# ashawkey/nerf2mesh

Hardware: AMD Instinct MI355X
Metric: train_samples_per_sec (higher is better)
Workload: dtype f32 march/composite, f16 autocast encode+MLP (reference -O recipe); 1 GPU; nerf_synthetic/lego stage-0 -O --bound 1 --dt_gamma 0, 800x800 x 100 synthetic views, num_points target 2^18/GPU (adaptive num_rays), occupancy refresh every 16 steps; diffuse_step=1000, refresh_steps_in_window=64, parallelism=single GPU, occupancy_refresh=single GPU, mlp=fused MFMA field kernels, driver=engine.Stage0Engine (fixed launch sequence), pretrain_steps=1000, params=18367240

## Files before the change

### include/n2m_hip.h

```cpp
#ifndef N2M_HIP_H
#define N2M_HIP_H

#include <stdint.h>

#ifdef __cplusplus
extern "C" {
#endif

#define N2M_ABI_VERSION 1

enum { N2M_F32 = 0, N2M_F16 = 1 };

enum {
    N2M_OK = 0,
    N2M_EINVAL = -1,
    N2M_ENULL = -2,
    N2M_EUNSUPPORTED = -3
};

int n2m_abi_version(void);
const char* n2m_last_error(void);


int n2m_near_far_from_aabb(const float* rays_o, const float* rays_d, const float* aabb, uint32_t N,
// ... 368 lines not shown
int n2m_freq_encode_forward(const float* inputs, uint32_t B, uint32_t D, uint32_t deg, uint32_t C,
                            float* outputs, void* stream);
int n2m_freq_encode_backward(const float* grad, const float* outputs, uint32_t B, uint32_t D, uint32_t deg,
                             uint32_t C, float* grad_inputs, void* stream);


int n2m_get_rays(const float* poses, const int64_t* cam, const int64_t* pix, uint32_t N, uint32_t H, uint32_t W,
                 float fx, float fy, float cx, float cy, const float* images, float* rays_o, float* rays_d,
                 float* rgba, void* stream);

int n2m_batch_rays(const float* poses, const float* uniforms, uint32_t V, uint32_t N, uint32_t H, uint32_t W, float fx, float fy, float cx,
                   float cy, const float* images, const float* aabb, float min_near, float* rays_o, float* rays_d, float* rgba,
                   float* nears, float* fars, float* noises, float* bg, int32_t* counter, void* stream);
int n2m_batch_rays_cnf(const float* poses, const float* uniforms, uint32_t V, uint32_t N, uint32_t H, uint32_t W, float fx, float fy, float cx,
                       float cy, const float* images, const float* aabb, float min_near, float* rays_o, float* rays_d, float* rgba,
                       float* nears, float* fars, float* noises, float* bg, int32_t* counter, const float* cam_near_far, void* stream);

int n2m_photo_loss_forward(const float* image, const float* weights_sum, const float* gt_rgba, const float* bg,
                           float bg_scalar, float lambda_rgb, float lambda_mask, uint32_t N, float* partial,
                           uint32_t* ticket, float* loss, void* stream);
int n2m_photo_loss_backward(const float* image, const float* weights_sum, const float* gt_rgba, const float* bg,
                            float bg_scalar, float lambda_rgb, float lambda_mask, uint32_t N,
                            const float* grad_loss, float* d_image, float* d_weights_sum, void* stream);

int n2m_composite_loss_train(const float* sigmas, const float* rgbs, const float* ts, const int32_t* rays, uint32_t M, uint32_t N,
                             float T_thresh, const float* gt_rgba, const float* bg, float bg_scalar, float lambda_rgb, float lambda_mask,
                             const float* grad_loss, float* weights_sum, float* image, float* grad_sigmas, float* grad_rgbs, float* partial,
                             uint32_t* ticket, float* loss, float* loss_sum, void* stream);
int n2m_composite_loss_train_ent(const float* sigmas, const float* rgbs, const float* ts, const int32_t* rays, uint32_t M, uint32_t N,
                                 float T_thresh, const float* gt_rgba, const float* bg, float bg_scalar, float lambda_rgb, float lambda_mask,
                                 const float* grad_loss, float* weights_sum, float* image, float* grad_sigmas, float* grad_rgbs, float* partial,
                                 uint32_t* ticket, float* loss, float* loss_sum, float lambda_entropy, void* stream);
int n2m_composite_loss_train_ex(const float* sigmas, const float* rgbs, const float* ts, const int32_t* rays, uint32_t M, uint32_t N,
                                float T_thresh, const float* gt_rgba, const float* bg, float bg_scalar, float lambda_rgb, float lambda_mask,
                                const float* grad_loss, float* weights_sum, float* image, float* grad_sigmas, float* grad_rgbs, float* partial,
                                uint32_t* ticket, float* loss, float* loss_sum, float lambda_entropy, int alpha_mode, void* stream);

int n2m_composite_live_counts(int32_t* live, uint32_t* block_live);
int n2m_sample_order_live_first(const int32_t* rays, const int32_t* live, const uint32_t* block_live, uint32_t N, uint32_t M,
                                uint32_t* perm, void* stream);
int n2m_grid_backward_sample_order(const uint32_t* perm);

int n2m_grid_backward_merge_levels(uint32_t levels);

#define N2M_ADAM_MAX 16
typedef struct {
    void* param[N2M_ADAM_MAX]; const void* grad[N2M_ADAM_MAX]; void* exp_avg[N2M_ADAM_MAX]; void* exp_avg_sq[N2M_ADAM_MAX];
    void* half_shadow[N2M_ADAM_MAX];
    uint32_t numel[N2M_ADAM_MAX]; float lr[N2M_ADAM_MAX]; int32_t grad_is_half[N2M_ADAM_MAX];
    int32_t shadow_mode[N2M_ADAM_MAX];
    int32_t clear_grad[N2M_ADAM_MAX];
    int32_t slot[N2M_ADAM_MAX];
    uint32_t count;
} N2mAdamDesc;
int n2m_adam_step(const N2mAdamDesc* desc, double beta1, double beta2, float eps, const float* scale,
                  const float* found_inf, const float* bias, void* stream);
#define N2M_EMA_MAX 16
typedef struct {
    void* shadow[N2M_EMA_MAX]; const void* param[N2M_EMA_MAX];
    uint32_t numel[N2M_EMA_MAX];
    uint32_t count;
} N2mEmaDesc;
int n2m_ema_update(const N2mEmaDesc* desc, float one_minus_decay, void* stream);

int n2m_scaler_update(float* scale, float* growth_tracker, float* found_inf, float* step, float* bias, double beta1,
                      double beta2, float growth_factor, float backoff_factor, float growth_interval, void* stream);
int n2m_scaler_update_slots(float* scale, float* growth_tracker, float* found_inf, float* steps, float* bias,
                            uint32_t participants, double beta1, double beta2, float growth_factor, float backoff_factor,
                            float growth_interval, void* stream);

int n2m_scaler_update_slots_loss(float* scale, float* growth_tracker, float* found_inf, float* steps, float* bias,
                                 uint32_t participants, double beta1, double beta2, float growth_factor, float backoff_factor,
                                 float growth_interval, const float* loss_partial, uint32_t n_partial, uint32_t n_rays, float* loss,
                                 float* loss_sum, void* stream);
int n2m_scaler_update_slots_loss2(float* scale, float* growth_tracker, float* found_inf, float* steps, float* bias,
                                  uint32_t participants, double beta1, double beta2, float growth_factor, float backoff_factor,
                                  float growth_interval, const float* loss_partial, uint32_t n_partial, uint32_t n_rays, float* loss,
                                  float* loss_sum, const float* extra_partial, uint32_t n_extra, float extra_scale, void* stream);
int n2m_scaler_update_slots_loss3(float* scale, float* growth_tracker, float* found_inf, float* steps, float* bias,
                                  uint32_t participants, double beta1, double beta2, float growth_factor, float backoff_factor,
                                  float growth_interval, const float* loss_partial, uint32_t n_partial, uint32_t n_rays, float* loss,
                                  float* loss_sum, const float* extra_partial, uint32_t n_extra, float extra_scale,
                                  const float* extra2_partial, uint32_t n_extra2, float extra2_scale, void* stream);

#define N2M_TAIL_TICKET_WORDS (64 * 32)
typedef struct {
    float* growth_tracker; float* steps;
    uint32_t participants; float growth_factor, backoff_factor, growth_interval;
    const float* loss_partial; uint32_t n_partial; uint32_t n_rays; float* loss; float* loss_sum;
    const float* extra_partial; uint32_t n_extra; float extra_scale;
    const float* extra2_partial; uint32_t n_extra2; float extra2_scale;
    uint32_t* ticket;
} N2mScalerTail;
int n2m_adam_step_scaler(const N2mAdamDesc* desc, double beta1, double beta2, float eps, float* scale, float* found_inf, float* bias,
                         const N2mScalerTail* tail, void* stream);

int n2m_sdf_offsets(const float* xyz, uint32_t M, float eps, float bound, float* pts, float* pts01, void* stream);
int n2m_sdf_alpha_forward(const float* sdf, const float* sdf6, const float* dirs, const float* ts, uint32_t M, const float* variance, float eps,
                          float cos_anneal_ratio, float* alpha, float* normal, float* eik_partial, void* stream);
int n2m_sdf_alpha_backward(const float* d_alpha, const float* sdf, const float* sdf6, const float* dirs, const float* ts, uint32_t M,
                           const float* variance, float eps, float cos_anneal_ratio, const float* seed, float eik_coef, float* d_sdf,
                           float* d_sdf6, float* var_partial, float* d_variance, float* found_inf, void* stream);


int n2m_sh_encode_forward(const float* inputs, float* outputs, uint32_t B, uint32_t D, uint32_t degree,
                          float* dy_dx, void* stream);

int n2m_sh_encode_backward(const float* grad, const float* inputs, uint32_t B, uint32_t D, uint32_t degree,
                           const float* dy_dx, float* grad_inputs, void* stream);


enum {
    N2M_K_GRID_FWD = 0, N2M_K_GRID_BWD, N2M_K_GRID_TV, N2M_K_MARCH_COUNT, N2M_K_MARCH_WRITE,
    N2M_K_COMPOSITE_FWD, N2M_K_COMPOSITE_BWD, N2M_K_NEAR_FAR, N2M_K_PACKBITS, N2M_K_MLP_FWD, N2M_K_MLP_BWD,
    N2M_K_RASTER, N2M_K_GRID_FWD_PACKED , N2M_K_ADAM,
    N2M_K_INTERP_FWD, N2M_K_INTERP_BWD, N2M_K_AA_FWD, N2M_K_AA_BWD, N2M_K_RASTER_BWD, N2M_K_COUNT
};
int n2m_prof_enable(int on);
int n2m_prof_reset(void);
int n2m_prof_read(int kernel_id, uint64_t* launches, double* total_ms, double* algo_bytes);
int n2m_prof_seen(int kernel_id, uint64_t* launches_seen);
const char* n2m_prof_name(int kernel_id);

int n2m_stream_copy(const void* src, void* dst, uint64_t bytes, uint32_t workgroups, void* stream);

#ifdef __cplusplus
}
#endif
#endif
```

### include/n2m_mlp.h

```cpp
#ifndef N2M_MLP_H
#define N2M_MLP_H

#include <stdint.h>

#ifdef __cplusplus
extern "C" {
#endif

int n2m_field_forward(const float* xyz, const float* dirs, const float* h1, const void* h2, const float* w_sigma0,
                      const float* w_sigma1, const float* w_color0, const float* w_color1, const float* w_color2,
                      const float* w_spec0, const float* w_spec1, uint32_t M, int shading, int normalize_dirs, float* sigma, float* rgb,
                      float* specular, void* stream);

int n2m_field_backward(const float* xyz, const float* dirs, const float* h1, const void* h2, const float* w_sigma0,
                       const float* w_sigma1, const float* w_color0, const float* w_color1, const float* w_color2,
                       const float* w_spec0, const float* w_spec1, uint32_t M, int shading, int normalize_dirs, const float* d_sigma,
                       const float* d_rgb, const float* d_specular, float* d_h1, void* d_h2, float* d_w_sigma0,
                       float* d_w_sigma1, float* d_w_color0, float* d_w_color1, float* d_w_color2, float* d_w_spec0,
                       float* d_w_spec1, float* found_inf, void* stream);

int n2m_field_forward_train(const float* xyz, const float* dirs, const float* h1, const void* h2, const float* w_sigma0,
                            const float* w_sigma1, const float* w_color0, const float* w_color1, const float* w_color2,
                            const float* w_spec0, const float* w_spec1, uint32_t M, int shading, int normalize_dirs, float* sigma, float* rgb,
                            float* specular, float* spec_sq_partial, void* stream);
int n2m_field_backward_train(const float* xyz, const float* dirs, const float* h1, const void* h2, const float* w_sigma0,
                             const float* w_sigma1, const float* w_color0, const float* w_color1, const float* w_color2,
                             const float* w_spec0, const float* w_spec1, uint32_t M, int shading, int normalize_dirs, const float* d_sigma,
                             const float* d_rgb, const float* d_specular, float* d_h1, void* d_h2, float* d_w_sigma0,
                             float* d_w_sigma1, float* d_w_color0, float* d_w_color1, float* d_w_color2, float* d_w_spec0,
                             float* d_w_spec1, float* found_inf, float spec_reg, const float* seed, void* stream);
uint32_t n2m_field_spec_partials(void);

#ifdef __cplusplus
}
#endif
#endif
```

### nerf2mesh_amd/_lib.py

```python
import ctypes
import os
import threading

_HERE = os.path.dirname(os.path.abspath(__file__))
LIB_PATH = os.environ.get("N2M_HIP_LIB") or os.path.join(_HERE, "lib", "libn2m_hip.so")

_u32, _i32, _f32, _vp, _int, _u64 = ctypes.c_uint32, ctypes.c_int32, ctypes.c_float, ctypes.c_void_p, ctypes.c_int, ctypes.c_uint64

SIGNATURES = {
    "n2m_near_far_from_aabb": [_vp, _vp, _vp, _u32, _f32, _vp, _vp, _vp],
    "n2m_sph_from_ray": [_vp, _vp, _f32, _u32, _vp, _vp],
    "n2m_morton3D": [_vp, _u32, _vp, _vp],
    "n2m_morton3D_invert": [_vp, _u32, _vp, _vp],
    "n2m_packbits": [_vp, _u32, _f32, _vp, _vp],
    "n2m_packbits_dev": [_vp, _u32, _vp, _vp, _vp],
    "n2m_flatten_rays": [_vp, _u32, _u32, _vp, _vp],
    "n2m_march_rays_train": [_vp, _vp, _vp, _f32, _int, _f32, _u32, _u32, _u32, _u32, _vp, _vp, _vp, _vp, _vp, _vp, _vp, _vp, _vp],
    "n2m_march_rays_train_write": [_vp, _vp, _vp, _f32, _int, _f32, _u32, _u32, _u32, _u32, _vp, _vp, _vp, _vp, _vp, _vp, _vp, _u32, _vp],
    "n2m_march_rays_train_fused": [_vp, _vp, _vp, _f32, _int, _f32, _u32, _u32, _u32, _u32, _vp, _vp, _vp, _vp, _vp, _vp, _vp, _vp, _u32, _vp, _u64, _vp],
    "n2m_march_fused_workspace_bytes": [_u32],
    "n2m_march_fallback_count": [_vp],
    "n2m_debug_fill_times": [_int, _vp],
    "n2m_stream_copy": [_vp, _vp, _u64, _u32, _vp],
    "n2m_composite_live_counts": [_vp, _vp],
# ... 33 lines not shown
                                             _vp, _f32, _f32, _f32, _vp, _vp, _f32, _f32, _int, _vp, _u64, _vp],
    "n2m_grid_encode_backward_binned_pair_half": [_vp, _vp, _vp, _vp, _vp, _vp, _u32, _u32, _u32, _f32, _u32, _u32, _int, _u32,
                                                  _vp, _f32, _f32, _f32, _vp, _vp, _f32, _f32, _int, _vp, _u64, _vp, _int],
    "n2m_sdf_fold_plan": [_vp, _u32, _f32, _f32, _u32, _u32, _f32, _u32, _int, _vp, _vp, _vp, _u32, _vp, _u32, _vp],
    "n2m_sdf_fold_gather": [_vp, _u32, _u32, _vp, _vp, _u32, _vp, _u32, _vp, _vp],
    "n2m_grid_encode_backward_binned_lists": [_vp, _vp, _u32, _vp, _vp, _u32, _u32, _u32, _f32, _u32, _u32, _int, _u32, _vp, _int, _vp, _u64, _vp],
    "n2m_grid_encode_backward_binned_pair_fold": [_vp, _vp, _vp, _vp, _vp, _vp, _u32, _u32, _u32, _f32, _u32, _u32, _int, _u32,
                                                  _vp, _f32, _f32, _f32, _vp, _vp, _f32, _f32, _int, _vp, _u64, _vp, _vp, _f32, _f32, _vp],
    "n2m_occupancy_update_partials": [_u32],
    "n2m_occupancy_points": [_vp, _vp, _vp, _f32, _f32, _vp, _u32, _vp],
    "n2m_occupancy_update": [_vp, _vp, _f32, _u32, _f32, _vp, _vp, _vp, _vp, _vp],
    "n2m_grid_pair_fuse_plan": [_u32, _u32, _vp, ctypes.POINTER(ctypes.c_uint32), ctypes.POINTER(ctypes.c_uint32)],
    "n2m_grid_encode_backward_binned_pair_adam": [_vp, _vp, _vp, _vp, _vp, _vp, _u32, _u32, _u32, _f32, _u32, _u32, _int, _u32,
                                                  _vp, _f32, _f32, _f32, _vp, _vp, _f32, _f32, _vp, _u64, _vp, _vp],
    "n2m_adam_fuse_restore": [_vp, _vp, _u32, _vp, _vp],
    "n2m_grid_tv_terms": [_vp, _vp, _vp, _u32, _u32, _f32, _u32, _u32, _int, _u32, _f32, _f32, _f32, _vp, _f32, _f32, _vp, _vp],
    "n2m_grid_encode_backward_binned_pair_tvt": [_vp, _vp, _vp, _vp, _vp, _vp, _u32, _u32, _u32, _f32, _u32, _u32, _int, _u32,
                                                 _vp, _vp, _f32, _f32, _int, _vp, _u64, _vp, _int],
    "n2m_grad_total_variation_binned": [_vp, _vp, _vp, _vp, _f32, _f32, _f32, _vp, _u32, _u32, _u32, _u32, _f32, _u32, _u32, _int, _vp, _u64, _vp],
    "n2m_marching_cubes_workspace_bytes": [_u32, _u32, _u32],
    "n2m_marching_cubes_count": [_vp, _u32, _u32, _u32, ctypes.c_double, _vp, _u64, _vp, _vp],
    "n2m_marching_cubes_emit": [_vp, _u32, _u32, _u32, ctypes.c_double, _vp, _u64, ctypes.c_double, ctypes.c_double, ctypes.c_double, _vp, _int,
                                _u32, _vp, _u32, _vp],
    "n2m_mesh_vertex_flags": [_vp, _u32, _vp, _vp, _vp, _u32, _vp, _vp],
    "n2m_mesh_quadrics": [_vp, _u32, _vp, _vp, _vp, _vp, _vp, ctypes.c_double, _vp, _vp],
    "n2m_mesh_edge_collapse_cost": [_vp, _vp, _vp, _vp, _u32, _vp, _vp, _vp, _vp, _vp, _vp, _int, _vp, _vp, _vp],
    "n2m_mesh_select_collapses": [_vp, _vp, _u32, _vp, _vp, _vp, _u32, _vp, _u64, _vp, _vp, _vp],
    "n2m_mesh_collapse_apply": [_vp, _u32, _vp, _vp, _vp, _vp, _u32, _vp, _u32, _vp, _vp, _vp],
    "n2m_mesh_compact_rows": [_vp, _u32, _u32, _u32, _vp, _vp, _vp, _vp],
    "n2m_mesh_mark_referenced": [_vp, _u32, _u32, _vp, _vp],
    "n2m_mesh_reindex": [_vp, _u32, _vp, _vp],
    "n2m_mesh_subdiv_mark": [_vp, _vp, _u32, _vp, _vp, ctypes.c_double, _u32, _vp, _vp],
    "n2m_mesh_subdiv_midpoints": [_vp, _u32, _vp, _u32, _vp, _vp, _vp],
    "n2m_mesh_subdiv_count": [_vp, _u32, _vp, _vp, _vp],
    "n2m_mesh_subdiv_emit": [_vp, _u32, _vp, _u32, _vp, _vp, _vp, _vp, _vp, _vp, _vp, _vp],
    "n2m_mesh_remesh_split_mark": [_vp, _vp, _u32, _u32, _vp, _vp, ctypes.c_double, _vp, _vp],
    "n2m_mesh_remesh_classify": [_vp, _u32, _vp, _vp, _u32, _vp, _vp, _vp, _vp, _vp, ctypes.c_double, _vp, _vp, _vp],
    "n2m_mesh_remesh_collapse_cost": [_vp, _vp, _vp, _vp, _u32, _vp, _vp, _vp, _vp, _vp, _vp, ctypes.c_double, ctypes.c_double, _vp, _vp, _vp],
    "n2m_mesh_remesh_flip_round": [_vp, _u32, _vp, _vp, _vp, _vp, _u32, _vp, _vp, _vp, _vp, _vp, _vp, _vp, _vp, _vp, _vp, _vp],
    "n2m_mesh_remesh_relax": [_vp, _u32, _vp, _vp, _vp, _vp, _vp, _vp, _vp, _vp, _vp, _vp, _vp],
    "n2m_mesh_remesh_relax_revert": [_vp, _vp, _u32, _vp, _u32, _vp, _vp, _vp, _vp, _vp],
    "n2m_mesh_bvh_morton": [_vp, _vp, _u32] + [ctypes.c_double] * 6 + [_vp, _vp],
    "n2m_mesh_bvh_hierarchy": [_vp, _u32, _vp, _vp, _vp],
    "n2m_mesh_bvh_refit": [_vp, _vp, _vp, _u32, _vp, _vp, _vp, _vp, _vp],
    "n2m_mesh_closest": [_vp, _vp, _vp, _u32, _vp, _vp, _vp, _u32, _int, ctypes.c_double, ctypes.c_double, _vp, _vp, _vp, _vp],
    "n2m_mesh_clean_cell_keys": [_vp, _u32, ctypes.c_double, ctypes.c_double, ctypes.c_double, ctypes.c_double, _i32, _i32, _i32, _vp, _vp],
    "n2m_mesh_clean_merge_round": [_vp, _u32, _vp, _vp, _vp, _i32, _i32, _i32, ctypes.c_double, _vp, _vp, _vp, _vp, _vp],
    "n2m_mesh_clean_repoint": [_vp, _u32, _vp, _vp, _vp],
    "n2m_mesh_clean_dup_null": [_vp, _vp, _u32, _vp, _vp, _vp, _vp],
    "n2m_mesh_clean_components": [_vp, _vp, _u32, _vp, _u32, _vp, _u64, _vp, _vp],
    "n2m_mesh_clean_component_filter": [_u32, _vp, _vp, _u32, _int, ctypes.c_double, _i32, _vp, _vp, _vp],
    "n2m_mesh_clean_nm_edge_init": [_vp, _vp, _u32, _vp, _vp, _vp, _vp, _vp, _vp],
    "n2m_mesh_clean_nm_edge_round": [_u32, _vp, _vp, _vp, _vp, _vp, _vp, _vp, _vp, _vp],
    "n2m_mesh_clean_fan_walk": [_vp, _u32, _u32, _vp, _vp, _vp, _vp, _vp, _vp, _vp, _vp],
    "n2m_mesh_clean_fan_split": [_vp, _u32, _vp, _vp, _vp, _vp, _vp, _u32, _vp],
    "n2m_uv_face_frames": [_vp, _vp, _u32, _vp, _vp, _vp, _vp, _vp, _vp],
    "n2m_uv_edge_faces": [_vp, _u32, _u32, _vp, _vp, _vp],
    "n2m_uv_relax_round": [_u32, _vp, _vp, _vp, _vp, _vp, _vp, _vp, ctypes.c_double, _vp, _vp, _vp, _vp],
    "n2m_uv_charts": [_u32, _vp, _vp, _vp, _vp, _vp, _vp, _vp, _vp, _vp, _vp],
    "n2m_uv_project": [_vp, _vp, _vp, _vp, _u32, _u32, _vp, _vp, _vp],
    "n2m_uv_sum_f64": [_vp, _u32, _vp, _vp],
    "n2m_uv_rects": [_vp, _u32, ctypes.c_double, _i32, _vp, _vp, _vp],
    "n2m_uv_shelf_pack": [_vp, _vp, _u32, _i32, _i32, _vp, _vp, _vp],
    "n2m_uv_write_vt": [_vp, _vp, _vp, _vp, _u32, ctypes.c_double, _i32, _i32, _i32, _vp, _vp],
    "n2m_uv_canvas_evict": [_vp, _vp, _u32, _i32, _i32, _vp, _vp, _vp],
    "n2m_uv_face_metrics": [_vp, _vp, _vp, _u32, _i32, _i32, _vp, _vp, _vp],
    "n2m_texture_pad_nearest": [_vp, _vp, _u32, _u32, _u32, _u32, _vp],
    "n2m_asset_shade": [_vp, _vp, _vp, _vp, _vp, _vp, _vp, _u32, _u32, _u32, _u32, _int, _int, _vp, _vp],
    "n2m_freq_encode_forward": [_vp, _u32, _u32, _u32, _u32, _vp, _vp],
    "n2m_freq_encode_backward": [_vp, _vp, _u32, _u32, _u32, _u32, _vp, _vp],
    "n2m_get_rays": [_vp, _vp, _vp, _u32, _u32, _u32, _f32, _f32, _f32, _f32, _vp, _vp, _vp, _vp, _vp],
    "n2m_batch_rays": [_vp, _vp, _u32, _u32, _u32, _u32, _f32, _f32, _f32, _f32, _vp, _vp, _f32, _vp, _vp, _vp, _vp, _vp, _vp, _vp, _vp, _vp],
    "n2m_batch_rays_cnf": [_vp, _vp, _u32, _u32, _u32, _u32, _f32, _f32, _f32, _f32, _vp, _vp, _f32, _vp, _vp, _vp, _vp, _vp, _vp, _vp, _vp, _vp, _vp],
    "n2m_adam_step": [_vp, ctypes.c_double, ctypes.c_double, _f32, _vp, _vp, _vp, _vp],
    "n2m_adam_step_scaler": [_vp, ctypes.c_double, ctypes.c_double, _f32, _vp, _vp, _vp, _vp, _vp],
    "n2m_ema_update": [_vp, _f32, _vp],
    "n2m_scaler_update": [_vp, _vp, _vp, _vp, _vp, ctypes.c_double, ctypes.c_double, _f32, _f32, _f32, _vp],
    "n2m_scaler_update_slots": [_vp, _vp, _vp, _vp, _vp, _u32, ctypes.c_double, ctypes.c_double, _f32, _f32, _f32, _vp],
    "n2m_scaler_update_slots_loss": [_vp, _vp, _vp, _vp, _vp, _u32, ctypes.c_double, ctypes.c_double, _f32, _f32, _f32, _vp, _u32, _u32, _vp, _vp, _vp],
    "n2m_scaler_update_slots_loss2": [_vp, _vp, _vp, _vp, _vp, _u32, ctypes.c_double, ctypes.c_double, _f32, _f32, _f32, _vp, _u32, _u32, _vp, _vp,
                                      _vp, _u32, _f32, _vp],
    "n2m_scaler_update_slots_loss3": [_vp, _vp, _vp, _vp, _vp, _u32, ctypes.c_double, ctypes.c_double, _f32, _f32, _f32, _vp, _u32, _u32, _vp, _vp,
                                      _vp, _u32, _f32, _vp, _u32, _f32, _vp],
    "n2m_sdf_offsets": [_vp, _u32, _f32, _f32, _vp, _vp, _vp],
    "n2m_sdf_alpha_forward": [_vp, _vp, _vp, _vp, _u32, _vp, _f32, _f32, _vp, _vp, _vp, _vp],
    "n2m_sdf_alpha_backward": [_vp, _vp, _vp, _vp, _vp, _u32, _vp, _f32, _f32, _vp, _f32, _vp, _vp, _vp, _vp, _vp, _vp],
    "n2m_photo_loss_forward": [_vp, _vp, _vp, _vp, _f32, _f32, _f32, _u32, _vp, _vp, _vp, _vp],
    "n2m_photo_loss_backward": [_vp, _vp, _vp, _vp, _f32, _f32, _f32, _u32, _vp, _vp, _vp, _vp],
    "n2m_sh_encode_forward": [_vp, _vp, _u32, _u32, _u32, _vp, _vp],
    "n2m_sh_encode_backward": [_vp, _vp, _u32, _u32, _u32, _vp, _vp, _vp],
    "n2m_field_forward": [_vp] * 11 + [_u32, _int, _int] + [_vp] * 4,
    "n2m_field_backward": [_vp] * 11 + [_u32, _int, _int] + [_vp] * 14,
    "n2m_field_forward_train": [_vp] * 11 + [_u32, _int, _int] + [_vp] * 5,
    "n2m_field_backward_train": [_vp] * 11 + [_u32, _int, _int] + [_vp] * 13 + [_f32, _vp, _vp],
    "n2m_field_spec_partials": [],
    "n2m_rasterize_forward": [_vp, _vp, _u32, _u32, _u32, _u32, _vp, _vp, _vp],
    "n2m_rasterize_backward": [_vp, _vp, _vp, _vp, _u32, _u32, _u32, _u32, _vp, _vp],
    "n2m_interpolate_forward": [_vp, _vp, _vp, _u32, _u32, _u32, _u32, _u32, _vp, _vp],
    "n2m_interpolate_backward": [_vp, _vp, _vp, _vp, _u32, _u32, _u32, _u32, _u32, _vp, _vp, _vp],
    "n2m_interpolate_backward_strided": [_vp, _vp, _vp, _vp, _u32, _u32, _u32, _u32, _u32, _u32, _vp, _vp, _vp],
    "n2m_antialias_build_topology": [_vp, _u32, _vp, _u32, _vp],
    "n2m_antialias_forward": [_vp, _vp, _vp, _vp, _vp, _u32, _u32, _u32, _u32, _u32, _u32, _vp, _vp],
    "n2m_antialias_backward": [_vp, _vp, _vp, _vp, _vp, _u32, _vp, _u32, _u32, _u32, _u32, _u32, _f32, _vp, _vp, _vp],
    "n2m_antialias_backward_seeded": [_vp, _vp, _vp, _vp, _vp, _u32, _vp, _u32, _u32, _u32, _u32, _u32, _f32, _vp, _vp, _vp],
    "n2m_to_clip": [_vp, _vp, _u32, _vp, _vp],
    "n2m_to_clip_backward": [_vp, _vp, _u32, _vp, _vp],
    "n2m_laplacian_forward": [_vp, _vp, _vp, _u32, _vp, _f32, _f32, _f32, _u32, _vp, _vp, _vp, _vp],
    "n2m_laplacian_backward": [_vp, _vp, _vp, _vp, _u32, _vp, _f32, _vp, _f32, _f32, _u32, _vp, _vp, _vp],
    "n2m_laplacian_backward_acc": [_vp, _vp, _vp, _vp, _u32, _vp, _f32, _vp, _f32, _f32, _u32, _vp, _vp, _vp],
    "n2m_gather_rows": [_vp, _vp, _u32, _u32, _vp, _vp],
    "n2m_gather_rows_strided": [_vp, _vp, _u32, _u32, _u32, _vp, _u32, _vp],
    "n2m_scatter_rows_strided": [_vp, _vp, _u32, _u32, _u32, _vp, _u32, _vp],
    "n2m_scatter_rows": [_vp, _vp, _u32, _u32, _vp, _vp],
    "n2m_stage1_head": [_vp, _vp, _vp, _u32, _u32, _u32, _vp, _vp, _f32, _f32, _f32, _vp, _vp, _vp, _vp, _vp, _vp, _vp, _vp, _vp, _vp, _int, _vp, _vp, _vp],
    "n2m_peer_alloc": [ctypes.c_size_t, _int, ctypes.POINTER(_vp)],
    "n2m_peer_free": [_vp],
    "n2m_peer_export": [_vp, _vp],
    "n2m_peer_import": [_vp, ctypes.POINTER(_vp)],
    "n2m_peer_unmap": [_vp],
    "n2m_peer_signal": [_vp, _u32, _vp],
    "n2m_peer_wait": [_vp, _u32, _u32, _u32, _u32, _vp, _vp],
    "n2m_peer_copy": [_vp, _vp, ctypes.c_size_t, _vp],
    "n2m_peer_reduce_slices": [_vp, _vp, _u32, _u32, _vp, _vp, _vp, _vp],
    "n2m_adam_step_peer": [_vp, ctypes.c_double, ctypes.c_double, _f32, _vp, _vp, _vp, _vp, _vp],
    "n2m_grid_backward_peer_route": [_vp],
    "n2m_prof_enable": [_int],
    "n2m_prof_reset": [],
    "n2m_prof_read": [_int, ctypes.POINTER(ctypes.c_uint64), ctypes.POINTER(ctypes.c_double), ctypes.POINTER(ctypes.c_double)],
    "n2m_prof_seen": [_int, ctypes.POINTER(ctypes.c_uint64)],
}

RESTYPES = {"n2m_occupancy_update_partials": _u32, "n2m_grid_binned_workspace_bytes": _u64, "n2m_grid_binned_pair_workspace_bytes": _u64, "n2m_march_fused_workspace_bytes": _u64,
            "n2m_marching_cubes_workspace_bytes": _u64, "n2m_field_spec_partials": _u32}

F32, F16 = 0, 1
ADAM_MAX = 16


class AdamDesc(ctypes.Structure):
    _fields_ = [("param", _vp * ADAM_MAX), ("grad", _vp * ADAM_MAX), ("exp_avg", _vp * ADAM_MAX), ("exp_avg_sq", _vp * ADAM_MAX),
                ("half_shadow", _vp * ADAM_MAX), ("numel", _u32 * ADAM_MAX), ("lr", _f32 * ADAM_MAX), ("grad_is_half", _i32 * ADAM_MAX),
                ("shadow_mode", _i32 * ADAM_MAX), ("clear_grad", _i32 * ADAM_MAX), ("slot", _i32 * ADAM_MAX), ("count", _u32)]


class ScalerTail(ctypes.Structure):
    _fields_ = [("growth_tracker", _vp), ("steps", _vp), ("participants", _u32), ("growth_factor", _f32), ("backoff_factor", _f32),
                ("growth_interval", _f32), ("loss_partial", _vp), ("n_partial", _u32), ("n_rays", _u32), ("loss", _vp), ("loss_sum", _vp),
                ("extra_partial", _vp), ("n_extra", _u32), ("extra_scale", _f32), ("extra2_partial", _vp), ("n_extra2", _u32),
                ("extra2_scale", _f32), ("ticket", _vp)]


EMA_MAX = 16


class EmaDesc(ctypes.Structure):
    _fields_ = [("shadow", _vp * EMA_MAX), ("param", _vp * EMA_MAX), ("numel", _u32 * EMA_MAX), ("count", _u32)]


ASSET_MAX = 8


class AssetTable(ctypes.Structure):
    _fields_ = [("feat0", _vp * ASSET_MAX), ("feat1", _vp * ASSET_MAX), ("Ht", _u32 * ASSET_MAX), ("Wt", _u32 * ASSET_MAX),
                ("face_begin", _u32 * ASSET_MAX), ("count", _u32)]


PEER_MAX = 8


class PeerPtrs(ctypes.Structure):
    _fields_ = [("ptr", _vp * PEER_MAX), ("count", _u32)]


class AdamPeer(ctypes.Structure):
    _fields_ = [("world", _u32), ("slots", (_vp * PEER_MAX) * 16), ("packed_local", _vp), ("packed_remote", _vp * PEER_MAX), ("n_remote", _u32)]


class PeerRoute(ctypes.Structure):
    _fields_ = [("world", _u32), ("split_row", _u32), ("rows_c", _u32), ("rows_f", _u32), ("g1", (_vp * PEER_MAX) * 2), ("g2", (_vp * PEER_MAX) * 2)]


class AdamFuse(ctypes.Structure):
    _fields_ = [("p_in", _vp * 2), ("m_in", _vp * 2), ("v_in", _vp * 2), ("p_out", _vp * 2), ("m_out", _vp * 2), ("v_out", _vp * 2),
                ("packed", _vp), ("first_level", _u32), ("lr", _f32 * 2), ("slot", _i32 * 2), ("beta1", ctypes.c_double),
                ("beta2", ctypes.c_double), ("eps", _f32), ("scale", _vp), ("bias", _vp)]


KERNEL_IDS = {"grid_encode_forward": 0, "grid_encode_backward": 1, "grad_total_variation": 2, "march_rays_train_count": 3,
              "march_rays_train_write": 4, "composite_rays_train_forward": 5, "composite_rays_train_backward": 6,
              "near_far_from_aabb": 7, "packbits": 8, "mlp_forward": 9, "mlp_backward": 10, "rasterize": 11,
              "grid_encode_forward_packed": 12, "adam_step": 13,
              "interpolate_forward": 14, "interpolate_backward": 15, "antialias_forward": 16, "antialias_backward": 17, "rasterize_backward": 18}

_lib = None


def lib():
    global _lib
    if _lib is None:
        import torch
        if not os.path.exists(LIB_PATH):
            raise RuntimeError(
                f"nerf2mesh_amd: {LIB_PATH} is missing -- build it with `python -m nerf2mesh_amd.build` "
                "(hipcc, gfx950). There is no CPU / PyTorch fallback for the hot path.")
        L = ctypes.CDLL(LIB_PATH)
        for name, argtypes in SIGNATURES.items():
            fn = getattr(L, name)
            fn.argtypes = argtypes
            fn.restype = RESTYPES.get(name, ctypes.c_int)
        L.n2m_last_error.restype = ctypes.c_char_p
        L.n2m_prof_name.restype = ctypes.c_char_p
        L.n2m_prof_name.argtypes = [_int]
        L.n2m_abi_version.restype = ctypes.c_int
        if L.n2m_abi_version() != 1:
            raise RuntimeError("nerf2mesh_amd: libn2m_hip.so ABI version mismatch")
        _lib = L
# ... 88 lines not shown
```

### nerf2mesh_amd/backends/__init__.py

```python
import os
import sys


def path():
    return os.path.dirname(os.path.abspath(__file__))


def install(fused_mlp=False):
    if fused_mlp:
        _fuse_on_import()
        track_torch_ema()
    p = path()
    if p not in sys.path:
        sys.path.insert(0, p)
    for name in ("mcubes", "nvdiffrast.torch", "nvdiffrast", "torch_scatter", "_raymarching_mob", "_gridencoder", "_shencoder", "_freqencoder"):
        m = sys.modules.get(name)
        if m is not None and getattr(m, "__n2m_stub__", False):
            del sys.modules[name]
    return p


def fuse_field(cls):
    import torch
    if getattr(cls, "_n2m_fused_field", False):
        return cls
    ref_forward, ref_density = cls.forward, cls.density

    def _prepare(self):
        ok = getattr(self, "_n2m_fuse_ok", None)
        if ok is None:
            try:
                e1, e2 = self.encoder, self.encoder_color
                shapes = [tuple(l.weight.shape) for m in (self.sigma_net, self.color_net, self.specular_net) for l in m.net]
                ok = (not getattr(self.opt, "tcnn", False) and getattr(self, "individual_dim", 0) == 0
                      and all(l.bias is None for m in (self.sigma_net, self.color_net, self.specular_net) for l in m.net)
                      and shapes == [(32, 19), (1, 32), (64, 35), (64, 64), (6, 64), (32, 6), (3, 32)]
                      and e1.embeddings.shape[1] == 1 and e2.embeddings.shape[1] == 2 and e1.num_levels == 16 and e2.num_levels == 16
                      and e1.input_dim == 3 and e2.input_dim == 3)
                if ok:
                    from nerf2mesh_amd.network import NeRFNetwork as _Ours
                    for e in (e1, e2):
                        if not hasattr(e, "host_offsets"):
                            e.host_offsets = [int(v) for v in e.offsets.detach().cpu().tolist()]
                    if not hasattr(type(self), "packed_tables"):
                        type(self).packed_tables = _Ours.packed_tables
                    if not hasattr(type(self), "invalidate_derived_copies"):
                        type(self).invalidate_derived_copies = _Ours.invalidate_derived_copies
                    from nerf2mesh_amd.network import derived_copy_holders
                    derived_copy_holders.add(self)
            except Exception:
                ok = False
            self._n2m_fuse_ok = ok
        return ok

    def forward(self, x, d, c=None, shading="full"):
        if c is None and x.is_cuda and shading in ("full", "diffuse", "specular") and _prepare(self):
            from nerf2mesh_amd.fused import fused_field
            lead = x.shape[:-1]
            sigma, color, specular = fused_field(self, x.reshape(-1, 3), d.reshape(-1, 3), shading)
            return sigma.view(lead), color.view(*lead, 3), (None if specular is None else specular.view(*lead, 3))
        return ref_forward(self, x, d, c, shading)

    def density(self, x):
        if x.is_cuda and not x.requires_grad and _prepare(self):
            from nerf2mesh_amd.fused import fused_density
            return {"sigma": fused_density(self, x.reshape(-1, 3)).view(x.shape[:-1])}
        return ref_density(self, x)

    forward.__doc__ = "nerf2mesh_amd.backends.fuse_field: fused MFMA field when covered, else " + (ref_forward.__qualname__)
    cls.forward, cls.density = forward, density
    cls._n2m_fused_field = True
    cls._n2m_reference_forward, cls._n2m_reference_density = ref_forward, ref_density
    return cls


def track_derived_copies(ema_cls):
    import functools
    if getattr(ema_cls, "_n2m_tracks_derived_copies", False):
        return ema_cls

    def written(ema, parameters):
        if parameters is not None:
            return parameters
        get = getattr(ema, "_get_parameters", None)
        if get is not None:
            return list(get(None))
        for name in ("_params", "params"):
            if isinstance(getattr(ema, name, None), (list, tuple)):
                return list(getattr(ema, name))
        return None

    def wrap(method):
        @functools.wraps(method)
        def wrapped(self, parameters=None):
            if parameters is not None:
                parameters = list(parameters)
            out = method(self, parameters)
            from nerf2mesh_amd.network import derived_copy_holders
            ps = written(self, parameters)
            ids = None if ps is None else {id(p) for p in ps}
            for model in list(derived_copy_holders):
                if ids is None or id(model.encoder.embeddings) in ids or id(model.encoder_color.embeddings) in ids:
                    model.invalidate_derived_copies()
            return out
        return wrapped

    ema_cls.copy_to, ema_cls.restore = wrap(ema_cls.copy_to), wrap(ema_cls.restore)
    ema_cls._n2m_tracks_derived_copies = True
    return ema_cls


def track_torch_ema():
    try:
        import torch_ema
    except ImportError:
        return False
    track_derived_copies(torch_ema.ExponentialMovingAverage)
    return True


def unfuse_field(cls):
    if getattr(cls, "_n2m_fused_field", False):
        cls.forward, cls.density = cls._n2m_reference_forward, cls._n2m_reference_density
        cls._n2m_fused_field = False
    return cls


def _fuse_on_import():
    m = sys.modules.get("nerf.network")
    if m is not None and hasattr(m, "NeRFNetwork"):
        fuse_field(m.NeRFNetwork)
        return
    import importlib.abc
    import importlib.util

    class _Hook(importlib.abc.MetaPathFinder):
        busy = False

        def find_spec(self, name, path_, target=None):
            if name != "nerf.network" or _Hook.busy:
                return None
            _Hook.busy = True
            try:
                spec = importlib.util.find_spec(name)
            finally:
                _Hook.busy = False
            if spec is None or spec.loader is None:
                return None
            loader, exec_module = spec.loader, spec.loader.exec_module

            def patched_exec(module):
                exec_module(module)
                if hasattr(module, "NeRFNetwork"):
                    fuse_field(module.NeRFNetwork)
            try:
                loader.exec_module = patched_exec
            except Exception:
                return None
            return spec

    if not any(type(h).__name__ == "_Hook" for h in sys.meta_path):
        sys.meta_path.insert(0, _Hook())
```

### nerf2mesh_amd/csrc/mlp.hip

```cpp
#include <map>
#include <mutex>

#include "n2m_common.hpp"
#include "../../include/n2m_mlp.h"

namespace {

typedef _Float16 h4 __attribute__((ext_vector_type(4)));
typedef float f16x __attribute__((ext_vector_type(16)));

#define MFMA(a, b, c) __builtin_amdgcn_mfma_f32_32x32x8f16((a), (b), (c), 0, 0, 0)
typedef _Float16 h8 __attribute__((ext_vector_type(8)));
#define MFMA16(a, b, c) __builtin_amdgcn_mfma_f32_32x32x16_f16((a), (b), (c), 0, 0, 0)

constexpr int P_S0 = 28, P_S1 = 36, P_C0 = 44, P_C1 = 68, P_C2 = 68, P_P0 = 12, P_P1 = 36;
constexpr int P_S1T = 12, P_S0T = 36, P_C2T = 12, P_C1T = 68, P_C0T = 68, P_P1T = 12, P_P0T = 36;
constexpr int O_S0 = 0;
constexpr int O_S1 = O_S0 + 32 * P_S0;
constexpr int O_C0 = O_S1 + 32 * P_S1;
constexpr int O_C1 = O_C0 + 64 * P_C0;
constexpr int O_C2 = O_C1 + 64 * P_C1;
constexpr int O_P0 = O_C2 + 32 * P_C2;
constexpr int O_P1 = O_P0 + 32 * P_P0;
constexpr int FWD_HALVES = O_P1 + 32 * P_P1;
constexpr int O_S1T = FWD_HALVES;
constexpr int O_S0T = O_S1T + 32 * P_S1T;
constexpr int O_C2T = O_S0T + 32 * P_S0T;
constexpr int O_C1T = O_C2T + 64 * P_C2T;
constexpr int O_C0T = O_C1T + 64 * P_C1T;
constexpr int O_P1T = O_C0T + 64 * P_C0T;
constexpr int O_P0T = O_P1T + 32 * P_P1T;
constexpr int ALL_W_HALVES = O_P0T + 32 * P_P0T;
constexpr int TILE_PITCH = 68;
constexpr int TILE_HALVES = 32 * TILE_PITCH;
constexpr int BWD_HALVES = ALL_W_HALVES + 4 * 2 * TILE_HALVES;
constexpr int BWD_PC_TILES_HALVES = ALL_W_HALVES + 4 * 4 * TILE_HALVES;
constexpr int BWD_PC_HALVES = BWD_PC_TILES_HALVES > 65536 ? BWD_PC_TILES_HALVES : 65536;

__device__ __forceinline__ int col_color0(int k) { return k < 32 ? 3 + k : (k < 35 ? k - 32 : -1); }
__device__ __forceinline__ int col_sigma0(int k) { return k < 16 ? 3 + k : (k < 19 ? k - 16 : -1); }
__device__ __forceinline__ int col_plain(int k, int in) { return k < in ? k : -1; }

enum Perm { PERM_PLAIN = 0, PERM_COLOR0 = 1, PERM_SIGMA0 = 2 };
__device__ __forceinline__ int col_of(int perm, int k, int in) {
    return perm == PERM_COLOR0 ? col_color0(k) : perm == PERM_SIGMA0 ? col_sigma0(k) : col_plain(k, in);
}

__device__ void stage_w(_Float16* dst, int pitch, const float* __restrict__ W, int out, int in, int m_pad, int k_pad, int perm) {
    for (int idx = threadIdx.x; idx < m_pad * k_pad; idx += blockDim.x) {
        const int m = idx / k_pad, k = idx - m * k_pad;
        const int c = col_of(perm, k, in);
        dst[m * pitch + k] = (_Float16)((m < out && c >= 0) ? W[m * in + c] : 0.0f);
    }
}
__device__ void stage_wt(_Float16* dst, int pitch, const float* __restrict__ W, int out, int in, int m_pad, int k_pad, int perm) {
    for (int idx = threadIdx.x; idx < m_pad * k_pad; idx += blockDim.x) {
        const int m = idx / k_pad, k = idx - m * k_pad;
        const int c = col_of(perm, m, in);
        dst[m * pitch + k] = (_Float16)((k < out && c >= 0) ? W[k * in + c] : 0.0f);
    }
}

struct FieldArgs {
    const float* xyz; const float* dirs; const float* h1; const _Float16* h2;
    const float* w[7];
    uint32_t M; int shading; int normalize_dirs;
    int raw_density;
    float* sigma; float* rgb; float* specular;
    const float* d_sigma; const float* d_rgb; const float* d_specular;
    float* d_h1; _Float16* d_h2; float* dw[7];
    float* found_inf;
    int dbg;
    float* dw_partial;
    float* spec_sq_partial;
    float spec_reg;
    const float* seed;
};
constexpr int kSpecPartials = 512;

template <int PERM>
__device__ __forceinline__ int logical_k(int c) {
    return PERM == PERM_COLOR0 ? (c < 3 ? 32 + c : c - 3) : PERM == PERM_SIGMA0 ? (c < 3 ? 16 + c : c - 3) : c;
}
template <int NT, int OUT, int IN>
struct WRegs { float v[(OUT * IN + NT - 1) / NT]; };
template <int NT, int OUT, int IN>
__device__ __forceinline__ void w_fetch(WRegs<NT, OUT, IN>& r, const float* __restrict__ W) {
#pragma unroll
    for (int i = 0; i < (OUT * IN + NT - 1) / NT; ++i) {
        const int e = (int)threadIdx.x + i * NT;
        r.v[i] = e < OUT * IN ? W[e] : 0.f;
    }
}
template <int NT, int OUT, int IN, int PERM, bool TR>
__device__ __forceinline__ void w_place(const WRegs<NT, OUT, IN>& r, _Float16* fwd, int pitch, _Float16* tr, int pitch_t) {
#pragma unroll
    for (int i = 0; i < (OUT * IN + NT - 1) / NT; ++i) {
        const int e = (int)threadIdx.x + i * NT;
        if (e < OUT * IN) {
            const int m = e / IN, k = logical_k<PERM>(e - m * IN);
            const _Float16 h = (_Float16)r.v[i];
            fwd[m * pitch + k] = h;
            if (TR) tr[k * pitch_t + m] = h;
        }
    }
}
template <int NT, bool TR, bool DO_DENSITY, bool DO_COLOR>
__device__ __forceinline__ void stage_images(_Float16* lds, const FieldArgs& a) {
    WRegs<NT, 32, 19> s0; WRegs<NT, 1, 32> s1; WRegs<NT, 64, 35> c0; WRegs<NT, 64, 64> c1; WRegs<NT, 6, 64> c2; WRegs<NT, 32, 6> p0; WRegs<NT, 3, 32> p1;
    const bool spec = DO_COLOR && a.shading != 0;
    if (DO_DENSITY) { w_fetch(s0, a.w[0]); w_fetch(s1, a.w[1]); }
    if (DO_COLOR) { w_fetch(c0, a.w[2]); w_fetch(c1, a.w[3]); w_fetch(c2, a.w[4]); }
    if (spec) { w_fetch(p0, a.w[5]); w_fetch(p1, a.w[6]); }
    const uint4 z = make_uint4(0u, 0u, 0u, 0u);
    for (int i = threadIdx.x; i < (TR ? ALL_W_HALVES : FWD_HALVES) / 8; i += NT) reinterpret_cast<uint4*>(lds)[i] = z;
    __syncthreads();
    if (DO_DENSITY) {
        w_place<NT, 32, 19, PERM_SIGMA0, TR>(s0, lds + O_S0, P_S0, lds + O_S0T, P_S0T);
        w_place<NT, 1, 32, PERM_PLAIN, TR>(s1, lds + O_S1, P_S1, lds + O_S1T, P_S1T);
    }
    if (DO_COLOR) {
        w_place<NT, 64, 35, PERM_COLOR0, TR>(c0, lds + O_C0, P_C0, lds + O_C0T, P_C0T);
        w_place<NT, 64, 64, PERM_PLAIN, TR>(c1, lds + O_C1, P_C1, lds + O_C1T, P_C1T);
        w_place<NT, 6, 64, PERM_PLAIN, TR>(c2, lds + O_C2, P_C2, lds + O_C2T, P_C2T);
    }
    if (spec) {
        w_place<NT, 32, 6, PERM_PLAIN, TR>(p0, lds + O_P0, P_P0, lds + O_P0T, P_P0T);
        w_place<NT, 3, 32, PERM_PLAIN, TR>(p1, lds + O_P1, P_P1, lds + O_P1T, P_P1T);
    }
    __syncthreads();
}

__device__ __forceinline__ h4 ld_a(const _Float16* W, int pitch, int mb, int kb, int lane) {
    return *reinterpret_cast<const h4*>(W + (32 * mb + (lane & 31)) * pitch + 8 * kb + 4 * (lane >> 5));
}

template <int MB, int KB>
__device__ __forceinline__ void ld_layer(h4 (&w)[MB][KB], const _Float16* W, int pitch, int lane) {
#pragma unroll
    for (int mb = 0; mb < MB; ++mb)
#pragma unroll
        for (int kb = 0; kb < KB; ++kb) w[mb][kb] = ld_a(W, pitch, mb, kb, lane);
}
__device__ __forceinline__ h8 cat8(const h4& lo, const h4& hi) { return __builtin_shufflevector(lo, hi, 0, 1, 2, 3, 4, 5, 6, 7); }
template <int MB, int KB>
__device__ __forceinline__ void mm_layer(f16x (&d)[MB], const h4 (&w)[MB][KB], const h4 (&b)[KB]) {
#pragma unroll
    for (int kb = 0; kb + 1 < KB; kb += 2)
#pragma unroll
        for (int mb = 0; mb < MB; ++mb) d[mb] = MFMA16(cat8(w[mb][kb], w[mb][kb + 1]), cat8(b[kb], b[kb + 1]), d[mb]);
    if (KB & 1) {
#pragma unroll
        for (int mb = 0; mb < MB; ++mb) d[mb] = MFMA(w[mb][KB - 1], b[KB - 1], d[mb]);
    }
}
template <int KB>
__device__ __forceinline__ f16x mm_k(const _Float16* W, int pitch, int mb, const h4 (&b)[KB], f16x acc, int lane) {
#pragma unroll
    for (int kb = 0; kb + 1 < KB; kb += 2)
        acc = MFMA16(cat8(ld_a(W, pitch, mb, kb, lane), ld_a(W, pitch, mb, kb + 1, lane)), cat8(b[kb], b[kb + 1]), acc);
    if (KB & 1) acc = MFMA(ld_a(W, pitch, mb, KB - 1, lane), b[KB - 1], acc);
    return acc;
}

__device__ __forceinline__ h4 zero4() { h4 z = {(_Float16)0, (_Float16)0, (_Float16)0, (_Float16)0}; return z; }
__device__ __forceinline__ f16x zero16() {
    f16x z;
#pragma unroll
    for (int i = 0; i < 16; ++i) z[i] = 0.f;
    return z;
}

typedef _Float16 h2v_t __attribute__((ext_vector_type(2)));
typedef short s2v_t __attribute__((ext_vector_type(2)));
typedef uint32_t u2v_t __attribute__((ext_vector_type(2)));
typedef float f2v_t __attribute__((ext_vector_type(2)));
__device__ __forceinline__ uint32_t cvt_pk(float a, float b) {
    const f2v_t v = {a, b};
    return __builtin_bit_cast(uint32_t, __builtin_convertvector(v, h2v_t));
}
__device__ __forceinline__ uint32_t relu_pk(uint32_t hh) {
    const s2v_t z = {0, 0};
    return __builtin_bit_cast(uint32_t, __builtin_elementwise_max(__builtin_bit_cast(s2v_t, hh), z));
}
__device__ __forceinline__ uint32_t positive_mask(uint32_t relu_out) {
    uint32_t m;
    asm("v_pk_sub_i16 %0, 0, %1\n\tv_pk_ashrrev_i16 %0, 15, %0 op_sel_hi:[0,1]" : "=v"(m) : "v"(relu_out));
    return m;
}
template <int Q>
__device__ __forceinline__ h4 relu_pack(const f16x& d) {
    u2v_t r;
    r.x = relu_pk(cvt_pk(d[4 * Q], d[4 * Q + 1]));
    r.y = relu_pk(cvt_pk(d[4 * Q + 2], d[4 * Q + 3]));
    return __builtin_bit_cast(h4, r);
}
template <int Q>
__device__ __forceinline__ h4 mask_pack(const f16x& d, const h4& fwd) {
    const u2v_t f = __builtin_bit_cast(u2v_t, fwd);
    u2v_t r;
    r.x = cvt_pk(d[4 * Q], d[4 * Q + 1]) & positive_mask(f.x);
    r.y = cvt_pk(d[4 * Q + 2], d[4 * Q + 3]) & positive_mask(f.y);
    return __builtin_bit_cast(h4, r);
}

__device__ __forceinline__ float sigmoid_h(float pre_acc) {
    const float x = (float)(_Float16)pre_acc;
    return (float)(_Float16)(1.0f / (1.0f + expf(-x)));
}


template <typename P>
__device__ __forceinline__ void load_dir(const FieldArgs& a, uint32_t s, P& bp) {
    float d0 = a.dirs[(size_t)s * 3], d1 = a.dirs[(size_t)s * 3 + 1], d2 = a.dirs[(size_t)s * 3 + 2];
    if (a.normalize_dirs) {
// ... 42 lines not shown
    float xyz[3], dir[3], dsig, drgb[3], dspec[3];
};
template <bool DO_DENSITY, bool DO_COLOR, bool BWD>
__device__ __forceinline__ void fetch_tile(const FieldArgs& a, uint32_t tile, int n, int g, RawTile& r) {
    const uint32_t s = tile * 32 + (uint32_t)n;
    const size_t Mz = a.M;
#pragma unroll
    for (int i = 0; i < 8; ++i) { r.h1v[i] = 0.f; r.h2v[i] = 0u; }
#pragma unroll
    for (int i = 0; i < 3; ++i) { r.xyz[i] = 0.f; r.dir[i] = 0.f; r.drgb[i] = 0.f; r.dspec[i] = 0.f; }
    r.dsig = 0.f;
    if (s >= a.M) return;
    if (DO_DENSITY) {
#pragma unroll
        for (int kb = 0; kb < 2; ++kb)
#pragma unroll
            for (int i = 0; i < 4; ++i) r.h1v[4 * kb + i] = a.h1[(size_t)(8 * kb + 4 * g + i) * Mz + s];
    }
    if (DO_COLOR) {
#pragma unroll
        for (int kb = 0; kb < 4; ++kb) {
            r.h2v[2 * kb] = *reinterpret_cast<const uint32_t*>(a.h2 + ((size_t)(4 * kb + 2 * g) * Mz + s) * 2);
            r.h2v[2 * kb + 1] = *reinterpret_cast<const uint32_t*>(a.h2 + ((size_t)(4 * kb + 2 * g + 1) * Mz + s) * 2);
        }
    }
    if (g == 0) {
#pragma unroll
        for (int i = 0; i < 3; ++i) r.xyz[i] = a.xyz[(size_t)s * 3 + i];
        if (DO_COLOR && a.shading != 0) {
#pragma unroll
            for (int i = 0; i < 3; ++i) r.dir[i] = a.dirs[(size_t)s * 3 + i];
        }
        if (BWD) {
            if (DO_DENSITY) r.dsig = a.d_sigma[s];
            if (DO_COLOR) {
#pragma unroll
                for (int i = 0; i < 3; ++i) r.drgb[i] = a.d_rgb[(size_t)s * 3 + i];
                if (a.d_specular && a.shading != 0) {
#pragma unroll
                    for (int i = 0; i < 3; ++i) r.dspec[i] = a.d_specular[(size_t)s * 3 + i];
                }
            }
        }
    }
}
__device__ __forceinline__ void settle_tile(RawTile& r) {
#pragma unroll
    for (int i = 0; i < 8; ++i) { asm volatile("" : "+v"(r.h1v[i])); asm volatile("" : "+v"(r.h2v[i])); }
#pragma unroll
    for (int i = 0; i < 3; ++i) { asm volatile("" : "+v"(r.xyz[i])); asm volatile("" : "+v"(r.dir[i])); asm volatile("" : "+v"(r.drgb[i])); asm volatile("" : "+v"(r.dspec[i])); }
    asm volatile("" : "+v"(r.dsig));
}
__device__ __forceinline__ void density_frags(const RawTile& r, h4 (&b)[3]) {
#pragma unroll
    for (int kb = 0; kb < 2; ++kb)
#pragma unroll
        for (int i = 0; i < 4; ++i) b[kb][i] = (_Float16)r.h1v[4 * kb + i];
    b[2] = zero4();
    b[2][0] = (_Float16)r.xyz[0]; b[2][1] = (_Float16)r.xyz[1]; b[2][2] = (_Float16)r.xyz[2];
}
__device__ __forceinline__ void color_frags(const RawTile& r, h4 (&b)[5]) {
#pragma unroll
    for (int kb = 0; kb < 4; ++kb) {
        const u2v_t v = {r.h2v[2 * kb], r.h2v[2 * kb + 1]};
        b[kb] = __builtin_bit_cast(h4, v);
    }
    b[4] = zero4();
    b[4][0] = (_Float16)r.xyz[0]; b[4][1] = (_Float16)r.xyz[1]; b[4][2] = (_Float16)r.xyz[2];
}
template <typename P>
__device__ __forceinline__ void dir_frag(const FieldArgs& a, const RawTile& r, P& bp) {
    float d0 = r.dir[0], d1 = r.dir[1], d2 = r.dir[2];
    if (a.normalize_dirs) {
        const float nn = sqrtf(fmaxf((d0 * d0 + d1 * d1) + d2 * d2, 1e-20f));
        d0 /= nn; d1 /= nn; d2 /= nn;
    }
    bp[0] = (_Float16)d0; bp[1] = (_Float16)d1; bp[2] = (_Float16)d2;
}

template <bool DO_DENSITY, bool DO_COLOR>
__global__ void __launch_bounds__(256) field_forward_kernel(FieldArgs a) {
    __builtin_amdgcn_s_setprio(3);
    extern __shared__ __attribute__((aligned(16))) _Float16 lds[];
    stage_images<256, false, DO_DENSITY, DO_COLOR>(lds, a);

    const int lane = threadIdx.x & 63, n = lane & 31, g = lane >> 5;
    const uint32_t wave = blockIdx.x * 4 + (threadIdx.x >> 6), n_waves = gridDim.x * 4;
    const uint32_t n_tiles = (a.M + 31) / 32;
    RawTile nxt;
    float spec_sq = 0.f;
    fetch_tile<DO_DENSITY, DO_COLOR, false>(a, wave, n, g, nxt);
    for (uint32_t tile = wave; tile < n_tiles; tile += n_waves) {
        const uint32_t s = tile * 32 + n;
        const bool valid = s < a.M;
        settle_tile(nxt);
        const RawTile cur = nxt;
        fetch_tile<DO_DENSITY, DO_COLOR, false>(a, tile + n_waves, n, g, nxt);
        if (DO_DENSITY) {
            h4 b0[3];
            density_frags(cur, b0);
            f16x d = zero16();
            d = mm_k<3>(lds + O_S0, P_S0, 0, b0, d, lane);
            const h4 b1[4] = {relu_pack<0>(d), relu_pack<1>(d), relu_pack<2>(d), relu_pack<3>(d)};
            f16x o = zero16();
            o = mm_k<4>(lds + O_S1, P_S1, 0, b1, o, lane);
            if (valid && g == 0) a.sigma[s] = a.raw_density ? (float)(_Float16)o[0] : expf((float)(_Float16)o[0]);
        }
        if (DO_COLOR) {
            h4 b0[5];
            color_frags(cur, b0);
            f16x d1[2] = {zero16(), zero16()};
#pragma unroll
            for (int mb = 0; mb < 2; ++mb)
                d1[mb] = mm_k<5>(lds + O_C0, P_C0, mb, b0, d1[mb], lane);
            const h4 b1[8] = {relu_pack<0>(d1[0]), relu_pack<1>(d1[0]), relu_pack<2>(d1[0]), relu_pack<3>(d1[0]),
                              relu_pack<0>(d1[1]), relu_pack<1>(d1[1]), relu_pack<2>(d1[1]), relu_pack<3>(d1[1])};
            f16x d2[2] = {zero16(), zero16()};
#pragma unroll
            for (int mb = 0; mb < 2; ++mb)
                d2[mb] = mm_k<8>(lds + O_C1, P_C1, mb, b1, d2[mb], lane);
            const h4 b2[8] = {relu_pack<0>(d2[0]), relu_pack<1>(d2[0]), relu_pack<2>(d2[0]), relu_pack<3>(d2[0]),
                              relu_pack<0>(d2[1]), relu_pack<1>(d2[1]), relu_pack<2>(d2[1]), relu_pack<3>(d2[1])};
            f16x d3 = zero16();
            d3 = mm_k<8>(lds + O_C2, P_C2, 0, b2, d3, lane);
            const float q0 = sigmoid_h(d3[0]), q1 = sigmoid_h(d3[1]), q2 = sigmoid_h(d3[2]), q3 = sigmoid_h(d3[3]);
            float cr = q0, cg = q1, cb = q2;
            if (a.shading != 0) {
                h4 bp = zero4();
                if (g == 0) {
                    if (valid) dir_frag(a, cur, bp);
                    bp[3] = (_Float16)q3;
                } else { bp[0] = (_Float16)q0; bp[1] = (_Float16)q1; }
                f16x p1 = MFMA(ld_a(lds + O_P0, P_P0, 0, 0, lane), bp, zero16());
                const h4 bq[4] = {relu_pack<0>(p1), relu_pack<1>(p1), relu_pack<2>(p1), relu_pack<3>(p1)};
                f16x p2 = zero16();
                p2 = mm_k<4>(lds + O_P1, P_P1, 0, bq, p2, lane);
                const float s0 = sigmoid_h(p2[0]), s1 = sigmoid_h(p2[1]), s2 = sigmoid_h(p2[2]);
                if (valid && g == 0 && a.specular) {
                    a.specular[(size_t)s * 3] = s0; a.specular[(size_t)s * 3 + 1] = s1; a.specular[(size_t)s * 3 + 2] = s2;
                }
                if (valid && g == 0) spec_sq += (s0 * s0 + s1 * s1) + s2 * s2;
                if (a.shading == 2) { cr = s0; cg = s1; cb = s2; }
                else {
                    cr = fminf(fmaxf((float)(_Float16)(s0 + q0), 0.f), 1.f);
                    cg = fminf(fmaxf((float)(_Float16)(s1 + q1), 0.f), 1.f);
                    cb = fminf(fmaxf((float)(_Float16)(s2 + q2), 0.f), 1.f);
                }
            }
            if (valid && g == 0 && a.rgb) {
                a.rgb[(size_t)s * 3] = cr; a.rgb[(size_t)s * 3 + 1] = cg; a.rgb[(size_t)s * 3 + 2] = cb;
            }
        }
    }
    if (DO_COLOR && a.spec_sq_partial) {
        __shared__ float spec_wave[4];
        const float w = n2m_wave_sum(spec_sq);
        if (lane == 0) spec_wave[threadIdx.x >> 6] = w;
        __syncthreads();
        if (threadIdx.x == 0) a.spec_sq_partial[blockIdx.x] = ((spec_wave[0] + spec_wave[1]) + spec_wave[2]) + spec_wave[3];
        if (blockIdx.x == 0)
            for (int i = (int)gridDim.x + (int)threadIdx.x; i < kSpecPartials; i += 256) a.spec_sq_partial[i] = 0.f;
    }
}

__device__ __forceinline__ void tile_put(_Float16* tile, int kb, const h4& f, int lane) {
    *reinterpret_cast<h4*>(tile + (lane & 31) * TILE_PITCH + 8 * kb + 4 * (lane >> 5)) = f;
}
// ... 279 lines not shown
                if (g == 0) dq3 = (float)(_Float16)dxp[3];
                else { dq0 = (float)(_Float16)dxp[0]; dq1 = (float)(_Float16)dxp[1]; }
            }
            h4 dc = zero4();
            if (g == 0) {
                dc[0] = (_Float16)(dq0 * q0 * (1.f - q0)); dc[1] = (_Float16)(dq1 * q1 * (1.f - q1));
                dc[2] = (_Float16)(dq2 * q2 * (1.f - q2)); dc[3] = (_Float16)(dq3 * q3 * (1.f - q3));
            } else { dc[0] = (_Float16)(dq0 * q0 * (1.f - q0)); dc[1] = (_Float16)(dq1 * q1 * (1.f - q1)); }
            if (!valid) dc = zero4();
            wave_lds_fence();
#pragma unroll
            for (int kb = 0; kb < 8; ++kb) tile_put(tX, kb, b2[kb], lane);
#pragma unroll
            for (int kb = 0; kb < 4; ++kb) tile_put(tY, kb, kb == 0 ? dc : zero4(), lane);
            wave_lds_fence();
            dw_tile<1, 2>(gC2, tY, tX, lane);
            f16x e2[2];
#pragma unroll
            for (int mb = 0; mb < 2; ++mb) e2[mb] = MFMA(ld_a(lds + O_C2T, P_C2T, mb, 0, lane), dc, zero16());
            const h4 dy2[8] = {mask_pack<0>(e2[0], b2[0]), mask_pack<1>(e2[0], b2[1]), mask_pack<2>(e2[0], b2[2]), mask_pack<3>(e2[0], b2[3]),
                               mask_pack<0>(e2[1], b2[4]), mask_pack<1>(e2[1], b2[5]), mask_pack<2>(e2[1], b2[6]), mask_pack<3>(e2[1], b2[7])};
            wave_lds_fence();
#pragma unroll
            for (int kb = 0; kb < 8; ++kb) { tile_put(tX, kb, b1[kb], lane); tile_put(tY, kb, dy2[kb], lane); }
            wave_lds_fence();
            dw_tile<2, 2>(gC1, tY, tX, lane);
            f16x e1[2] = {zero16(), zero16()};
#pragma unroll
            for (int mb = 0; mb < 2; ++mb)
#pragma unroll
                for (int kb = 0; kb < 8; ++kb) e1[mb] = MFMA(ld_a(lds + O_C1T, P_C1T, mb, kb, lane), dy2[kb], e1[mb]);
            const h4 dy1[8] = {mask_pack<0>(e1[0], b1[0]), mask_pack<1>(e1[0], b1[1]), mask_pack<2>(e1[0], b1[2]), mask_pack<3>(e1[0], b1[3]),
                               mask_pack<0>(e1[1], b1[4]), mask_pack<1>(e1[1], b1[5]), mask_pack<2>(e1[1], b1[6]), mask_pack<3>(e1[1], b1[7])};
            wave_lds_fence();
#pragma unroll
            for (int kb = 0; kb < 8; ++kb) { tile_put(tY, kb, dy1[kb], lane); tile_put(tX, kb, kb < 5 ? b0[kb] : zero4(), lane); }
            wave_lds_fence();
            dw_tile<2, 2>(gC0, tY, tX, lane);
            f16x e0 = zero16();
#pragma unroll
            for (int kb = 0; kb < 8; ++kb) e0 = MFMA(ld_a(lds + O_C0T, P_C0T, 0, kb, lane), dy1[kb], e0);
            if (valid) {
                typedef _Float16 h2v __attribute__((ext_vector_type(2)));
#pragma unroll
                for (int r = 0; r < 16; r += 2) {
                    const int row = 8 * (r >> 2) + 4 * g + (r & 3);
                    h2v v;
                    v.x = (_Float16)e0[r]; v.y = (_Float16)e0[r + 1];
                    *reinterpret_cast<h2v*>(a.d_h2 + ((size_t)(row >> 1) * Mz + s) * 2) = v;
                }
            }
        }
    }

    __syncthreads();
    float* stage = reinterpret_cast<float*>(lds);
    auto reduce = [&](auto& acc, int out_pad, int in_pad, float* dW, int out, int in, int k_real, int perm) {
        for (int i = threadIdx.x; i < out_pad * in_pad; i += blockDim.x) stage[i] = 0.f;
        __syncthreads();
        dw_to_lds(stage, in_pad, acc, lane);
        __syncthreads();
        dw_flush(dW, stage, in_pad, out, in, k_real, perm, a.found_inf);
        __syncthreads();
    };
    if (DO_DENSITY) {
        reduce(gS1, 32, 32, a.dw[1], 1, 32, 32, PERM_PLAIN);
        reduce(gS0, 32, 32, a.dw[0], 32, 19, 19, PERM_SIGMA0);
    }
    if (DO_COLOR) {
        reduce(gC2, 32, 64, a.dw[4], 6, 64, 64, PERM_PLAIN);
        reduce(gC1, 64, 64, a.dw[3], 64, 64, 64, PERM_PLAIN);
        reduce(gC0, 64, 64, a.dw[2], 64, 35, 35, PERM_COLOR0);
        if (a.shading != 0) {
            reduce(gP1, 32, 32, a.dw[6], 3, 32, 32, PERM_PLAIN);
            reduce(gP0, 32, 32, a.dw[5], 32, 6, 6, PERM_PLAIN);
        }
    }
}

template <bool DO_DENSITY, bool DO_COLOR>
__global__ void __launch_bounds__(512) __attribute__((amdgpu_waves_per_eu(2, 2))) field_backward_pc_kernel(FieldArgs a) {
    __builtin_amdgcn_s_setprio(3);
    extern __shared__ __attribute__((aligned(16))) _Float16 lds[];
    stage_images<512, true, DO_DENSITY, DO_COLOR>(lds, a);

    const int lane = threadIdx.x & 63, n = lane & 31, g = lane >> 5, wid = threadIdx.x >> 6;
    const int pair = wid & 3;
    const bool producer = wid < 4;
    _Float16* const tbase = lds + ALL_W_HALVES + pair * 4 * TILE_HALVES;
    auto TX = [&](uint32_t st) { return tbase + (st & 1u) * 2 * TILE_HALVES; };
    auto TY = [&](uint32_t st) { return tbase + (st & 1u) * 2 * TILE_HALVES + TILE_HALVES; };
    const uint32_t n_tiles = (a.dbg & 1) ? 0u : (a.M + 31) / 32;
    const size_t Mz = a.M;
    uint32_t st = 0;
    const float spec_k = a.spec_reg != 0.f ? *a.seed * a.spec_reg : 0.f;

    f16x gS0[1][1] = {{zero16()}}, gS1[1][1] = {{zero16()}};
    f16x gC0[2][2], gC1[2][2], gC2[1][2], gP0[1][1] = {{zero16()}}, gP1[1][1] = {{zero16()}};
#pragma unroll
    for (int i = 0; i < 2; ++i)
#pragma unroll
        for (int j = 0; j < 2; ++j) { gC0[i][j] = zero16(); gC1[i][j] = zero16(); gC2[0][j] = zero16(); }

    if (producer) {
    RawTile nxt;
    fetch_tile<DO_DENSITY, DO_COLOR, true>(a, blockIdx.x * 4 + pair, n, g, nxt);
    for (uint32_t base = blockIdx.x * 4; base < n_tiles; base += gridDim.x * 4) {
        const uint32_t tile = base + pair;
        const uint32_t s = tile * 32 + n;
        const bool valid = s < a.M;
        settle_tile(nxt);
        const RawTile cur = nxt;
        fetch_tile<DO_DENSITY, DO_COLOR, true>(a, tile + gridDim.x * 4, n, g, nxt);
        if (DO_DENSITY) {
            h4 b0[3];
            density_frags(cur, b0);
            f16x d = zero16();
            d = mm_k<3>(lds + O_S0, P_S0, 0, b0, d, lane);
            const h4 b1[4] = {relu_pack<0>(d), relu_pack<1>(d), relu_pack<2>(d), relu_pack<3>(d)};
            f16x o = zero16();
            o = mm_k<4>(lds + O_S1, P_S1, 0, b1, o, lane);
            h4 dy1 = zero4();
            if (valid && g == 0) {
                const float pre = (float)(_Float16)o[0];
                dy1[0] = a.raw_density ? (_Float16)cur.dsig : (_Float16)(cur.dsig * expf(fminf(fmaxf(pre, -15.f), 15.f)));
            }
#pragma unroll
            for (int kb = 0; kb < 4; ++kb) { tile_put(TX(st), kb, b1[kb], lane); tile_put(TY(st), kb, kb == 0 ? dy1 : zero4(), lane); }
            __syncthreads(); ++st;
            const f16x dh = MFMA(ld_a(lds + O_S1T, P_S1T, 0, 0, lane), dy1, zero16());
            const h4 dy0[4] = {mask_pack<0>(dh, b1[0]), mask_pack<1>(dh, b1[1]), mask_pack<2>(dh, b1[2]), mask_pack<3>(dh, b1[3])};
#pragma unroll
            for (int kb = 0; kb < 4; ++kb) { tile_put(TY(st), kb, dy0[kb], lane); tile_put(TX(st), kb, kb < 3 ? b0[kb] : zero4(), lane); }
            __syncthreads(); ++st;
            f16x dx = zero16();
            dx = mm_k<4>(lds + O_S0T, P_S0T, 0, dy0, dx, lane);
            if (valid) {
#pragma unroll
                for (int r = 0; r < 8; ++r) {
                    const int row = 8 * (r >> 2) + 4 * g + (r & 3);
                    a.d_h1[(size_t)row * Mz + s] = (float)(_Float16)dx[r];
                }
            }
        }
        if (DO_COLOR) {
            h4 b0[5];
            h4 wC0[2][5], wC1[2][8], wC2[1][8];
            ld_layer(wC0, lds + O_C0, P_C0, lane);
            color_frags(cur, b0);
            ld_layer(wC1, lds + O_C1, P_C1, lane);
            __builtin_amdgcn_sched_barrier(0);
            f16x d1[2] = {zero16(), zero16()};
            mm_layer(d1, wC0, b0);
            ld_layer(wC2, lds + O_C2, P_C2, lane);
            __builtin_amdgcn_sched_barrier(0);
            const h4 b1[8] = {relu_pack<0>(d1[0]), relu_pack<1>(d1[0]), relu_pack<2>(d1[0]), relu_pack<3>(d1[0]),
                              relu_pack<0>(d1[1]), relu_pack<1>(d1[1]), relu_pack<2>(d1[1]), relu_pack<3>(d1[1])};
            f16x d2[2] = {zero16(), zero16()};
            mm_layer(d2, wC1, b1);
            const h4 b2[8] = {relu_pack<0>(d2[0]), relu_pack<1>(d2[0]), relu_pack<2>(d2[0]), relu_pack<3>(d2[0]),
                              relu_pack<0>(d2[1]), relu_pack<1>(d2[1]), relu_pack<2>(d2[1]), relu_pack<3>(d2[1])};
            f16x d3v[1] = {zero16()};
            mm_layer(d3v, wC2, b2);
            const f16x d3 = d3v[0];
            const float q0 = sigmoid_h(d3[0]), q1 = sigmoid_h(d3[1]), q2 = sigmoid_h(d3[2]), q3 = sigmoid_h(d3[3]);

            float gr = 0.f, gg = 0.f, gb = 0.f, es0 = 0.f, es1 = 0.f, es2 = 0.f;
// ... 89 lines not shown
        }
    }
    }
    else
    for (uint32_t base = blockIdx.x * 4; base < n_tiles; base += gridDim.x * 4) {
        if (DO_DENSITY) {
            __syncthreads(); dw_tile<1, 1, true>(gS1, TY(st), TX(st), lane); ++st;
            __syncthreads(); dw_tile<1, 1, true>(gS0, TY(st), TX(st), lane); ++st;
        }
        if (DO_COLOR) {
            if (a.shading != 0) {
                __syncthreads(); dw_tile<1, 1, true>(gP1, TY(st), TX(st), lane); ++st;
                __syncthreads(); dw_tile<1, 1, true>(gP0, TY(st), TX(st), lane); ++st;
            }
            __syncthreads(); dw_tile<1, 2, true>(gC2, TY(st), TX(st), lane); ++st;
            __syncthreads(); dw_tile<2, 2, true>(gC1, TY(st), TX(st), lane); ++st;
            __syncthreads(); dw_tile<2, 2, true>(gC0, TY(st), TX(st), lane); ++st;
        }
    }

    __syncthreads();
    float* stage = reinterpret_cast<float*>(lds);
    float* const part_row = a.dw_partial + (size_t)blockIdx.x * kDwTotal;
    if (a.dbg & 2) return;
    auto put = [&](auto& acc, int base, int out_pad, int in_pad, int total) {
        if (!producer) dw_to_copy(stage + pair * total + base, in_pad, acc, lane);
    };
    auto sum = [&](int base, int total, int in_pad, int mat, int out, int in, int k_real, int perm) {
        dw_store_partial(part_row + kDwOff[mat], stage + base, total, in_pad, out, in, k_real, perm);
    };
    if (DO_COLOR) {
        put(gC1, 0, 64, 64, 8192); put(gC0, 4096, 64, 64, 8192);
        __syncthreads();
        sum(0, 8192, 64, 3, 64, 64, 64, PERM_PLAIN); sum(4096, 8192, 64, 2, 64, 35, 35, PERM_COLOR0);
        __syncthreads();
    }
    constexpr int kSmall = 6144;
    if (DO_COLOR) {
        put(gC2, 0, 32, 64, kSmall);
        if (a.shading != 0) { put(gP1, 4096, 32, 32, kSmall); put(gP0, 5120, 32, 32, kSmall); }
    }
    if (DO_DENSITY) { put(gS1, 2048, 32, 32, kSmall); put(gS0, 3072, 32, 32, kSmall); }
    __syncthreads();
    if (DO_COLOR) {
        sum(0, kSmall, 64, 4, 6, 64, 64, PERM_PLAIN);
        if (a.shading != 0) { sum(4096, kSmall, 32, 6, 3, 32, 32, PERM_PLAIN); sum(5120, kSmall, 32, 5, 32, 6, 6, PERM_PLAIN); }
    }
    if (DO_DENSITY) { sum(2048, kSmall, 32, 1, 1, 32, 32, PERM_PLAIN); sum(3072, kSmall, 32, 0, 32, 19, 19, PERM_SIGMA0); }
}

int check_field(const char* fn, const float* xyz, const float* h1, const float* const* w, bool density, int shading) {
    N2M_REQUIRE(shading >= 0 && shading <= 2, N2M_EINVAL, "%s: shading must be 0 (diffuse), 1 (full) or 2 (specular)", fn);
    N2M_REQUIRE(xyz, N2M_ENULL, "%s: xyz is NULL", fn);
    if (density) N2M_REQUIRE(h1 && w[0] && w[1], N2M_ENULL, "%s: density branch needs h1 and sigma_net weights", fn);
    return 0;
}

float* dw_scratch(hipStream_t s) {
    static std::mutex mu;
    static std::map<std::pair<int, hipStream_t>, float*> bufs;
    std::lock_guard<std::mutex> lk(mu);
    int dev = 0;
    if (hipGetDevice(&dev) != hipSuccess) return nullptr;
    const auto key = std::make_pair(dev, s);
    auto it = bufs.find(key);
    if (it != bufs.end()) return it->second;
    float* p = nullptr;
    if (hipMalloc((void**)&p, (size_t)256 * kDwTotal * sizeof(float)) != hipSuccess) return nullptr;
    bufs[key] = p;
    return p;
}

uint32_t persistent_grid(uint32_t M) {
    const uint32_t tiles = (M + 31) / 32;
    const uint32_t need = (tiles + 3) / 4;
    return need < 256u ? (need ? need : 1u) : 256u;
}

}

static int field_forward_impl(const float* xyz, const float* dirs, const float* h1, const void* h2, const float* w_sigma0,
                                 const float* w_sigma1, const float* w_color0, const float* w_color1, const float* w_color2,
                                 const float* w_spec0, const float* w_spec1, uint32_t M, int shading, int normalize_dirs, float* sigma, float* rgb,
                                 float* specular, float* spec_sq_partial, void* stream) {
    const float* w[7] = {w_sigma0, w_sigma1, w_color0, w_color1, w_color2, w_spec0, w_spec1};
    const bool density = sigma != nullptr;
    if (int rc = check_field("field_forward", xyz, h1, w, density, shading)) return rc;
    const bool color = rgb != nullptr;
    N2M_REQUIRE(density || color, N2M_ENULL, "field_forward: both sigma and rgb are NULL");
    if (color) {
        N2M_REQUIRE(h2 && w[2] && w[3] && w[4], N2M_ENULL, "field_forward: colour branch needs h2 and color_net weights");
        if (shading != 0) N2M_REQUIRE(dirs && w[5] && w[6], N2M_ENULL, "field_forward: shading != 0 needs dirs and specular_net weights");
    }
    if (M == 0) return 0;
    FieldArgs a{};
    a.xyz = xyz; a.dirs = dirs; a.h1 = h1; a.h2 = (const _Float16*)h2; a.normalize_dirs = normalize_dirs & 1; a.raw_density = (normalize_dirs >> 1) & 1;
    for (int i = 0; i < 7; ++i) a.w[i] = w[i];
    a.M = M; a.shading = shading; a.sigma = sigma; a.rgb = rgb; a.specular = specular;
    a.spec_sq_partial = (color && shading != 0) ? spec_sq_partial : nullptr;
    hipStream_t s = (hipStream_t)stream;
    N2M_PROF_K(N2M_K_MLP_FWD, s, (double)M * (12 + 64 + 4 + (color ? 64 + 12 + 12 + 12 : 0)));
    const size_t smem = (size_t)FWD_HALVES * 2;
    if (color && density) N2M_LAUNCH((field_forward_kernel<true, true>), persistent_grid(M) * 2, 256, smem, s, a);
    else if (color) N2M_LAUNCH((field_forward_kernel<false, true>), persistent_grid(M) * 2, 256, smem, s, a);
    else N2M_LAUNCH((field_forward_kernel<true, false>), persistent_grid(M) * 2, 256, smem, s, a);
    N2M_CHECK_LAUNCH();
    return 0;
}

extern "C" int n2m_field_forward(const float* xyz, const float* dirs, const float* h1, const void* h2, const float* w_sigma0,
                                 const float* w_sigma1, const float* w_color0, const float* w_color1, const float* w_color2,
                                 const float* w_spec0, const float* w_spec1, uint32_t M, int shading, int normalize_dirs, float* sigma, float* rgb,
                                 float* specular, void* stream) {
    return field_forward_impl(xyz, dirs, h1, h2, w_sigma0, w_sigma1, w_color0, w_color1, w_color2, w_spec0, w_spec1, M, shading, normalize_dirs,
                              sigma, rgb, specular, nullptr, stream);
}
extern "C" int n2m_field_forward_train(const float* xyz, const float* dirs, const float* h1, const void* h2, const float* w_sigma0,
                                       const float* w_sigma1, const float* w_color0, const float* w_color1, const float* w_color2,
                                       const float* w_spec0, const float* w_spec1, uint32_t M, int shading, int normalize_dirs, float* sigma,
                                       float* rgb, float* specular, float* spec_sq_partial, void* stream) {
    return field_forward_impl(xyz, dirs, h1, h2, w_sigma0, w_sigma1, w_color0, w_color1, w_color2, w_spec0, w_spec1, M, shading, normalize_dirs,
                              sigma, rgb, specular, spec_sq_partial, stream);
}
extern "C" uint32_t n2m_field_spec_partials(void) { return (uint32_t)kSpecPartials; }

static int field_backward_impl(const float* xyz, const float* dirs, const float* h1, const void* h2, const float* w_sigma0,
                                  const float* w_sigma1, const float* w_color0, const float* w_color1, const float* w_color2,
                                  const float* w_spec0, const float* w_spec1, uint32_t M, int shading, int normalize_dirs, const float* d_sigma,
                                  const float* d_rgb, const float* d_specular, float* d_h1, void* d_h2, float* d_w_sigma0,
                                  float* d_w_sigma1, float* d_w_color0, float* d_w_color1, float* d_w_color2, float* d_w_spec0,
                                  float* d_w_spec1, float* found_inf, float spec_reg, const float* seed, void* stream) {
    const float* w[7] = {w_sigma0, w_sigma1, w_color0, w_color1, w_color2, w_spec0, w_spec1};
    float* dw[7] = {d_w_sigma0, d_w_sigma1, d_w_color0, d_w_color1, d_w_color2, d_w_spec0, d_w_spec1};
    const bool density = d_sigma != nullptr;
    if (int rc = check_field("field_backward", xyz, h1, w, density, shading)) return rc;
    if (density) N2M_REQUIRE(d_h1 && dw[0] && dw[1], N2M_ENULL, "field_backward: density gradients are NULL");
    const bool color = d_rgb != nullptr;
    N2M_REQUIRE(density || color, N2M_ENULL, "field_backward: both d_sigma and d_rgb are NULL");
    if (color) {
        N2M_REQUIRE(h2 && d_h2 && w[2] && w[3] && w[4] && dw[2] && dw[3] && dw[4], N2M_ENULL, "field_backward: colour branch tensors are NULL");
        if (shading != 0) N2M_REQUIRE(dirs && w[5] && w[6] && dw[5] && dw[6], N2M_ENULL, "field_backward: specular branch tensors are NULL");
    }
    if (M == 0) return 0;
    static bool attr_set = false;
    if (!attr_set) {
        (void)hipFuncSetAttribute((const void*)field_backward_kernel<true, true>, hipFuncAttributeMaxDynamicSharedMemorySize, BWD_HALVES * 2);
        (void)hipFuncSetAttribute((const void*)field_backward_kernel<true, false>, hipFuncAttributeMaxDynamicSharedMemorySize, BWD_HALVES * 2);
        (void)hipFuncSetAttribute((const void*)field_backward_kernel<false, true>, hipFuncAttributeMaxDynamicSharedMemorySize, BWD_HALVES * 2);
        (void)hipFuncSetAttribute((const void*)field_backward_pc_kernel<true, true>, hipFuncAttributeMaxDynamicSharedMemorySize, BWD_PC_HALVES * 2);
        (void)hipFuncSetAttribute((const void*)field_backward_pc_kernel<true, false>, hipFuncAttributeMaxDynamicSharedMemorySize, BWD_PC_HALVES * 2);
        (void)hipFuncSetAttribute((const void*)field_backward_pc_kernel<false, true>, hipFuncAttributeMaxDynamicSharedMemorySize, BWD_PC_HALVES * 2);
        attr_set = true;
    }
    FieldArgs a{};
    a.xyz = xyz; a.dirs = dirs; a.h1 = h1; a.h2 = (const _Float16*)h2; a.normalize_dirs = normalize_dirs & 1; a.raw_density = (normalize_dirs >> 1) & 1;
    for (int i = 0; i < 7; ++i) { a.w[i] = w[i]; a.dw[i] = dw[i]; }
    a.M = M; a.shading = shading;
    a.spec_reg = (color && shading != 0 && seed) ? spec_reg : 0.f; a.seed = seed;
    a.d_sigma = d_sigma; a.d_rgb = d_rgb; a.d_specular = d_specular; a.d_h1 = d_h1; a.d_h2 = (_Float16*)d_h2; a.found_inf = found_inf;
    static const int dbg = getenv("N2M_FIELD_DEBUG") ? atoi(getenv("N2M_FIELD_DEBUG")) : 0;
    a.dbg = dbg;
    hipStream_t s = (hipStream_t)stream;
    N2M_PROF_K(N2M_K_MLP_BWD, s, (double)M * (12 + 64 + 4 + 64 + (color ? 64 + 12 + 24 + 64 : 0)));
    static const bool single_wave = getenv("N2M_FIELD_BWD_SINGLE") != nullptr;
    if (!single_wave) {
        const size_t smem = (size_t)BWD_PC_HALVES * 2;
        const uint32_t grid = persistent_grid(M);
        float* part = dw_scratch(s);
        N2M_REQUIRE(part != nullptr, (int)hipErrorOutOfMemory, "field_backward: no memory for the weight-gradient scratch");
        a.dw_partial = part;
        if (color && density) N2M_LAUNCH((field_backward_pc_kernel<true, true>), grid, 512, smem, s, a);
        else if (color) N2M_LAUNCH((field_backward_pc_kernel<false, true>), grid, 512, smem, s, a);
        else N2M_LAUNCH((field_backward_pc_kernel<true, false>), grid, 512, smem, s, a);
        N2M_CHECK_LAUNCH();
        DwOut o;
        for (int i = 0; i < 7; ++i) o.dw[i] = dw[i];
        const uint32_t mask = (density ? 0x03u : 0u) | (color ? 0x1Cu : 0u) | (color && shading != 0 ? 0x60u : 0u);
        if (!(dbg & 2)) N2M_LAUNCH(dw_finalize_kernel, (kDwTotal + 63) / 64, 1024, 0, s, part, grid, o, mask, found_inf);
        N2M_CHECK_LAUNCH();
        return 0;
    }
    const size_t smem = (size_t)BWD_HALVES * 2;
    if (color && density) N2M_LAUNCH((field_backward_kernel<true, true>), persistent_grid(M), 256, smem, s, a);
    else if (color) N2M_LAUNCH((field_backward_kernel<false, true>), persistent_grid(M), 256, smem, s, a);
    else N2M_LAUNCH((field_backward_kernel<true, false>), persistent_grid(M), 256, smem, s, a);
    N2M_CHECK_LAUNCH();
    return 0;
}

extern "C" int n2m_field_backward(const float* xyz, const float* dirs, const float* h1, const void* h2, const float* w_sigma0,
                                  const float* w_sigma1, const float* w_color0, const float* w_color1, const float* w_color2,
                                  const float* w_spec0, const float* w_spec1, uint32_t M, int shading, int normalize_dirs, const float* d_sigma,
                                  const float* d_rgb, const float* d_specular, float* d_h1, void* d_h2, float* d_w_sigma0,
                                  float* d_w_sigma1, float* d_w_color0, float* d_w_color1, float* d_w_color2, float* d_w_spec0,
                                  float* d_w_spec1, float* found_inf, void* stream) {
    return field_backward_impl(xyz, dirs, h1, h2, w_sigma0, w_sigma1, w_color0, w_color1, w_color2, w_spec0, w_spec1, M, shading, normalize_dirs,
                               d_sigma, d_rgb, d_specular, d_h1, d_h2, d_w_sigma0, d_w_sigma1, d_w_color0, d_w_color1, d_w_color2, d_w_spec0,
                               d_w_spec1, found_inf, 0.f, nullptr, stream);
}
extern "C" int n2m_field_backward_train(const float* xyz, const float* dirs, const float* h1, const void* h2, const float* w_sigma0,
                                        const float* w_sigma1, const float* w_color0, const float* w_color1, const float* w_color2,
                                        const float* w_spec0, const float* w_spec1, uint32_t M, int shading, int normalize_dirs,
                                        const float* d_sigma, const float* d_rgb, const float* d_specular, float* d_h1, void* d_h2,
                                        float* d_w_sigma0, float* d_w_sigma1, float* d_w_color0, float* d_w_color1, float* d_w_color2,
                                        float* d_w_spec0, float* d_w_spec1, float* found_inf, float spec_reg, const float* seed, void* stream) {
    return field_backward_impl(xyz, dirs, h1, h2, w_sigma0, w_sigma1, w_color0, w_color1, w_color2, w_spec0, w_spec1, M, shading, normalize_dirs,
                               d_sigma, d_rgb, d_specular, d_h1, d_h2, d_w_sigma0, d_w_sigma1, d_w_color0, d_w_color1, d_w_color2, d_w_spec0,
                               d_w_spec1, found_inf, spec_reg, seed, stream);
}
```

### nerf2mesh_amd/csrc/step_helpers.hip

```cpp
#include <string.h>

#include "n2m_common.hpp"
#include "../../include/n2m_peer.h"

namespace {

struct RayTerm {
    float e[3];
    float m;
    float bg[3];
};

__device__ __forceinline__ RayTerm ray_term(const float* __restrict__ image, const float* __restrict__ wsum,
                                            const float* __restrict__ gt, const float* __restrict__ bg, float bg_scalar, uint32_t r) {
    RayTerm t;
    const float4 g = *reinterpret_cast<const float4*>(gt + (size_t)r * 4);
    const float a = g.w, ws = wsum[r];
    const float gc[3] = {g.x, g.y, g.z};
#pragma unroll
    for (int c = 0; c < 3; ++c) {
        t.bg[c] = bg ? bg[(size_t)r * 3 + c] : bg_scalar;
        const float target = gc[c] * a + t.bg[c] * (1.0f - a);
        const float pred = image[(size_t)r * 3 + c] + (1.0f - ws) * t.bg[c];
        t.e[c] = pred - target;
    }
    t.m = ws - a;
    return t;
}

__global__ void __launch_bounds__(256)
photo_loss_forward_kernel(const float* __restrict__ image, const float* __restrict__ wsum, const float* __restrict__ gt,
                          const float* __restrict__ bg, float bg_scalar, float lambda_rgb, float lambda_mask, uint32_t N,
                          float* __restrict__ partial, uint32_t* __restrict__ ticket, float* __restrict__ loss) {
    __shared__ float wave_sum[4];
    __shared__ bool last;
    const uint32_t r = blockIdx.x * 256 + threadIdx.x, lane = threadIdx.x & 63u, wid = threadIdx.x >> 6;
    float l = 0.0f;
    if (r < N) {
        const RayTerm t = ray_term(image, wsum, gt, bg, bg_scalar, r);
        l = lambda_rgb * ((t.e[0] * t.e[0] + t.e[1] * t.e[1] + t.e[2] * t.e[2]) / 3.0f) + lambda_mask * (t.m * t.m);
    }
    l = n2m_wave_sum(l);
    if (lane == 0) wave_sum[wid] = l;
    __syncthreads();
    if (threadIdx.x == 0) {
        partial[blockIdx.x] = (wave_sum[0] + wave_sum[1]) + (wave_sum[2] + wave_sum[3]);
        __threadfence();
        last = atomicAdd(ticket, 1u) == gridDim.x - 1;
    }
    __syncthreads();
    if (last) {
        __threadfence();
        float s = 0.0f;
        for (uint32_t i = threadIdx.x; i < gridDim.x; i += 256) s += __hip_atomic_load(&partial[i], __ATOMIC_RELAXED, __HIP_MEMORY_SCOPE_AGENT);
        s = n2m_wave_sum(s);
        if (lane == 0) wave_sum[wid] = s;
        __syncthreads();
        if (threadIdx.x == 0) {
            *loss = ((wave_sum[0] + wave_sum[1]) + (wave_sum[2] + wave_sum[3])) / (float)N;
            *ticket = 0;
        }
    }
}

__global__ void __launch_bounds__(256)
photo_loss_backward_kernel(const float* __restrict__ image, const float* __restrict__ wsum, const float* __restrict__ gt,
                           const float* __restrict__ bg, float bg_scalar, float lambda_rgb, float lambda_mask, uint32_t N,
                           const float* __restrict__ grad_loss, float* __restrict__ d_image, float* __restrict__ d_wsum) {
    const uint32_t r = blockIdx.x * 256 + threadIdx.x;
    if (r >= N) return;
    const float g = *grad_loss / (float)N;
    const RayTerm t = ray_term(image, wsum, gt, bg, bg_scalar, r);
    float dw = g * lambda_mask * 2.0f * t.m;
#pragma unroll
    for (int c = 0; c < 3; ++c) {
        const float dp = g * lambda_rgb * (2.0f * t.e[c] / 3.0f);
        d_image[(size_t)r * 3 + c] = dp;
        dw -= dp * t.bg[c];
    }
    d_wsum[r] = dw;
}

template <int S>
__global__ void __launch_bounds__(256)
stage1_head_kernel(const float* __restrict__ aa_alpha , const float* __restrict__ aa_rgb ,
// ... 1040 lines not shown
            float acc = 0.0f;
            for (uint32_t i = s; i < n_partial; i += blockDim.x) acc += loss_partial[i];
            acc = n2m_wave_sum(acc);
            if ((s & 63u) == 0u) wave_part[s >> 6] = acc;
        }
        ok = *found_inf == 0.0f;
        __syncthreads();
        if (s == 0) {
            for (uint32_t w = 0; w < (blockDim.x + 63u) / 64u; ++w) {
                if (loss_partial) tot_part += wave_part[w];
                if (extra_partial) tot_extra += wave_extra[w];
                if (extra2_partial) tot_extra2 += wave_extra2[w];
            }
        }
    }
    if (loss_partial && s == 0) {
        float v = tot_part * inv_rays;
        if (extra_partial) v += tot_extra * extra_scale;
        if (extra2_partial) v += tot_extra2 * extra2_scale;
        if (loss) *loss = v;
        if (loss_sum) *loss_sum += v;
    }
    if (s == 0) {
        if (!ok) {
            if (scale) *scale *= backoff_factor;
            if (growth_tracker) *growth_tracker = 0.0f;
        } else if (growth_tracker) {
            const float g = *growth_tracker + 1.0f;
            if (g >= growth_interval) {
                const float ns = *scale * growth_factor;
                if (scale && ns <= 3.0e38f) *scale = ns;
                *growth_tracker = 0.0f;
            } else {
                *growth_tracker = g;
            }
        }
        *found_inf = 0.0f;
    }
    if (s <= N2M_ADAM_MAX) {
        if (ok && (s == 0 || ((participants >> (s - 1u)) & 1u))) steps[s] += 1.0f;
        const double t = (double)steps[s] + 1.0;
        bias[2u * s] = (float)(1.0 - pow(beta1, t));
        bias[2u * s + 1u] = (float)sqrt(1.0 - pow(beta2, t));
    }
}

__global__ void scaler_update_slots_kernel(float* scale, float* growth_tracker, float* found_inf, float* steps ,
                                           float* bias , uint32_t participants, double beta1, double beta2,
                                           float growth_factor, float backoff_factor, float growth_interval,
                                           const float* __restrict__ loss_partial, uint32_t n_partial, float inv_rays,
                                           float* __restrict__ loss, float* __restrict__ loss_sum,
                                           const float* __restrict__ extra_partial, uint32_t n_extra, float extra_scale,
                                           const float* __restrict__ extra2_partial = nullptr, uint32_t n_extra2 = 0, float extra2_scale = 0.0f) {
    __builtin_amdgcn_s_setprio(3);
    scaler_update_slots_body<false>(scale, growth_tracker, found_inf, steps, bias, participants, beta1, beta2, growth_factor, backoff_factor, growth_interval,
                             loss_partial, n_partial, inv_rays, loss, loss_sum, extra_partial, n_extra, extra_scale, extra2_partial, n_extra2, extra2_scale);
}

extern "C" int n2m_scaler_update_slots(float* scale, float* growth_tracker, float* found_inf, float* steps, float* bias,
                                       uint32_t participants, double beta1, double beta2, float growth_factor, float backoff_factor,
                                       float growth_interval, void* stream) {
    N2M_REQUIRE(found_inf != nullptr && steps != nullptr && bias != nullptr, N2M_ENULL, "scaler_update_slots: NULL found_inf / steps / bias");
    scaler_update_slots_kernel<<<1, 64, 0, (hipStream_t)stream>>>(scale, growth_tracker, found_inf, steps, bias, participants, beta1, beta2,
                                                                  growth_factor, backoff_factor, growth_interval, nullptr, 0u, 0.0f, nullptr, nullptr, nullptr, 0u, 0.0f);
    N2M_CHECK_LAUNCH();
    return 0;
}

extern "C" int n2m_scaler_update_slots_loss3(float* scale, float* growth_tracker, float* found_inf, float* steps, float* bias,
                                            uint32_t participants, double beta1, double beta2, float growth_factor, float backoff_factor,
                                            float growth_interval, const float* loss_partial, uint32_t n_partial, uint32_t n_rays, float* loss,
                                            float* loss_sum, const float* extra_partial, uint32_t n_extra, float extra_scale, const float* extra2_partial,
                                             uint32_t n_extra2, float extra2_scale, void* stream) {
    N2M_REQUIRE(found_inf != nullptr && steps != nullptr && bias != nullptr, N2M_ENULL, "scaler_update_slots: NULL found_inf / steps / bias");
    N2M_REQUIRE(loss_partial != nullptr && n_rays > 0, N2M_EINVAL, "scaler_update_slots_loss: needs the loss partials and the ray count");
    scaler_update_slots_kernel<<<1, 256, 0, (hipStream_t)stream>>>(scale, growth_tracker, found_inf, steps, bias, participants, beta1, beta2,
                                                                  growth_factor, backoff_factor, growth_interval, loss_partial, n_partial,
                                                                  1.0f / (float)n_rays, loss, loss_sum, extra_partial, extra_partial ? n_extra : 0u, extra_scale,
                                                                  extra2_partial, extra2_partial ? n_extra2 : 0u, extra2_scale);
    N2M_CHECK_LAUNCH();
    return 0;
}

extern "C" int n2m_scaler_update_slots_loss2(float* scale, float* growth_tracker, float* found_inf, float* steps, float* bias,
                                             uint32_t participants, double beta1, double beta2, float growth_factor, float backoff_factor,
                                             float growth_interval, const float* loss_partial, uint32_t n_partial, uint32_t n_rays, float* loss,
                                             float* loss_sum, const float* extra_partial, uint32_t n_extra, float extra_scale, void* stream) {
    return n2m_scaler_update_slots_loss3(scale, growth_tracker, found_inf, steps, bias, participants, beta1, beta2, growth_factor, backoff_factor,
                                         growth_interval, loss_partial, n_partial, n_rays, loss, loss_sum, extra_partial, n_extra, extra_scale,
                                         nullptr, 0u, 0.0f, stream);
}

extern "C" int n2m_scaler_update_slots_loss(float* scale, float* growth_tracker, float* found_inf, float* steps, float* bias,
                                            uint32_t participants, double beta1, double beta2, float growth_factor, float backoff_factor,
                                            float growth_interval, const float* loss_partial, uint32_t n_partial, uint32_t n_rays, float* loss,
                                            float* loss_sum, void* stream) {
    return n2m_scaler_update_slots_loss2(scale, growth_tracker, found_inf, steps, bias, participants, beta1, beta2, growth_factor, backoff_factor,
                                         growth_interval, loss_partial, n_partial, n_rays, loss, loss_sum, nullptr, 0u, 0.0f, stream);
}

extern "C" int n2m_scaler_update(float* scale, float* growth_tracker, float* found_inf, float* step, float* bias, double beta1,
                                 double beta2, float growth_factor, float backoff_factor, float growth_interval, void* stream) {
    N2M_REQUIRE(found_inf != nullptr, N2M_ENULL, "scaler_update: found_inf is NULL");
    scaler_update_kernel<<<1, 1, 0, (hipStream_t)stream>>>(scale, growth_tracker, found_inf, step, bias, beta1, beta2, growth_factor,
                                                           backoff_factor, growth_interval);
    N2M_CHECK_LAUNCH();
    return 0;
}

struct EmaTensors {
    uint64_t shadow[N2M_EMA_MAX], param[N2M_EMA_MAX];
    uint32_t n[N2M_EMA_MAX], first_block[N2M_EMA_MAX + 1];
    uint32_t count;
};

__global__ void __launch_bounds__(256) ema_update_kernel(EmaTensors t, float one_minus_decay) {
    uint32_t k = 0;
    while (k + 1 < t.count && blockIdx.x >= t.first_block[k + 1]) ++k;
    const uint32_t i0 = ((blockIdx.x - t.first_block[k]) * 256u + threadIdx.x) * 4u;
    const uint32_t n = t.n[k];
    if (i0 >= n) return;
    float* __restrict__ S = reinterpret_cast<float*>(t.shadow[k]);
    const float* __restrict__ P = reinterpret_cast<const float*>(t.param[k]);
    typedef float f4v __attribute__((ext_vector_type(4)));
    if (i0 + 4u <= n && (((t.shadow[k] | t.param[k]) & 15u) == 0)) {
        f4v s = __builtin_nontemporal_load(reinterpret_cast<const f4v*>(S + i0));
        const f4v p = __builtin_nontemporal_load(reinterpret_cast<const f4v*>(P + i0));
        s.x = s.x - (s.x - p.x) * one_minus_decay; s.y = s.y - (s.y - p.y) * one_minus_decay;
        s.z = s.z - (s.z - p.z) * one_minus_decay; s.w = s.w - (s.w - p.w) * one_minus_decay;
        __builtin_nontemporal_store(s, reinterpret_cast<f4v*>(S + i0));
    } else {
        for (uint32_t e = 0; e < 4u && i0 + e < n; ++e) S[i0 + e] = S[i0 + e] - (S[i0 + e] - P[i0 + e]) * one_minus_decay;
    }
}

extern "C" int n2m_ema_update(const N2mEmaDesc* d, float one_minus_decay, void* stream) {
    N2M_REQUIRE(d != nullptr, N2M_ENULL, "ema_update: NULL descriptor");
    N2M_REQUIRE(d->count >= 1 && d->count <= N2M_EMA_MAX, N2M_EINVAL, "ema_update: 1..%d tensors per call (got %u)", N2M_EMA_MAX, d->count);
    N2M_REQUIRE(one_minus_decay >= 0.0f && one_minus_decay <= 1.0f, N2M_EINVAL, "ema_update: 1 - decay = %g outside [0, 1]", (double)one_minus_decay);
    EmaTensors t;
    t.count = d->count;
    uint32_t blocks = 0;
    for (uint32_t k = 0; k < d->count; ++k) {
        N2M_REQUIRE(d->shadow[k] && d->param[k], N2M_ENULL, "ema_update: NULL tensor %u", k);
        N2M_REQUIRE((((uintptr_t)d->shadow[k] | (uintptr_t)d->param[k]) & 3u) == 0, N2M_EINVAL, "ema_update: tensor %u is not 4-byte aligned", k);
        N2M_REQUIRE(d->shadow[k] != d->param[k], N2M_EINVAL, "ema_update: tensor %u: shadow and parameter are the same memory", k);
        t.shadow[k] = (uint64_t)(uintptr_t)d->shadow[k];
        t.param[k] = (uint64_t)(uintptr_t)d->param[k];
        t.n[k] = d->numel[k];
        t.first_block[k] = blocks;
        blocks += (d->numel[k] + 1023u) / 1024u;
    }
    t.first_block[d->count] = blocks;
    if (blocks == 0) return 0;
    ema_update_kernel<<<blocks, 256, 0, (hipStream_t)stream>>>(t, one_minus_decay);
    N2M_CHECK_LAUNCH();
    return 0;
}
```

### nerf2mesh_amd/engine.py

```python
import ctypes
import os
import time

import numpy as np
import torch

from . import _lib as L
from . import raymarching, synthetic
from .fused import SHADING, _affine
from .gridencoder import _host_offsets, same_geometry
from .optim import FusedAdamAMP

_p = L.ptr


def _shard_refresh_default():
    from .parallel import shard_refresh_default
    return shard_refresh_default()


def lr_lambda(it, iters):
    return 0.01 + 0.99 * (it / 500) if it <= 500 else 0.1 ** ((it - 500) / (iters - 500))


# ... 18 lines not shown
        self.one_pass = False
        self.host_count = torch.empty(1, dtype=torch.int32, pin_memory=True)
        self.count_ready = torch.cuda.Event()
        self.written = torch.cuda.Event()
        self.spec = False
        self.index = 0
        self.M = None
        self.loss = torch.empty(1, dtype=torch.float32, device=dev)
        self.samples = None
        self.cap_m = 0
        self.N = 0
        self.args = None
        self.refreshed = False


class Stage0Engine:
    def __init__(self, model, opt, poses, device, rank=0, world_size=1, seed=0, ema_decay=0.95):
        self.model, self.opt, self.device = model.to(device), opt, torch.device(device)
        dev = self.device
        assert dev.type == "cuda", "the step executor drives HIP kernels: no CPU path"
        if bool(opt.sdf) and world_size > 1:
            raise ValueError("Stage0Engine runs the SDF recipe on one rank; use trainer.Stage0Trainer for multi-rank SDF training")
        if not self.supported(model, opt):
            raise ValueError("Stage0Engine covers the fused recipes (fused_mlp, fp16, no individual codes, power-of-two "
                             "bound, shared encoder geometry); use trainer.Stage0Trainer for other configurations")
        L.lib()
        self.poses = poses.to(dev).float().contiguous()
        self.rank, self.world = rank, world_size
        self.global_step = 0
        self.num_rays = opt.num_rays
        self.gen = torch.Generator(device=dev)
        self.gen.manual_seed(seed + rank)
        self.optimizer = FusedAdamAMP(model.get_params(opt.lr), eps=1e-15, amp=True)
        self.ema = None
        self.epoch_len = max(1, int(poses.shape[0]))
        if ema_decay is not None:
            from .ema import ExponentialMovingAverage
            self.ema = ExponentialMovingAverage(model.parameters(), decay=ema_decay)
        self.images = None
        self.scene = getattr(opt, "scene", "lego")
        self.boxes = synthetic.boxes(dev, self.scene)
        self.cam_near_far = synthetic.cam_near_far(self.poses, self.scene) if getattr(opt, "enable_cam_near_far", False) else None
        self.samples_seen = self.rays_seen = 0
        self.last_num_points = 0
        self._loss_pending, self._loss_sum = [], torch.zeros(1, device=dev)
        self.sync = None
        if world_size > 1:
            from .parallel import GradSync
            self.sync = GradSync(model, world_size)
            self.model.refresh_shard = (rank, world_size) if _shard_refresh_default() else None
        self.side = L.side_stream(dev, slot=2)
        self.tv_stream = L.side_stream(dev, slot=3, priority=int(os.environ.get("N2M_TV_PRIO", "0")))
        self.tv_split = os.environ.get("N2M_TV_SPLIT", "0") == "1"
        self.tv_at = int(os.environ.get("N2M_TV_AT", "0"))
        self.split_backward = True
        self.overlap = True
        self.single_pass = os.environ.get("N2M_MARCH_PASSES", "1") != "2"
        self.marker_at = int(os.environ.get("N2M_MARKER_AT", "0"))
        self.tv_corners = (os.environ.get("N2M_TV_CORNERS", "0") == "1" and world_size == 1 and not opt.sdf and opt.lambda_tv > 0
                           and not self.tv_split)
        self.tv_fwd = (os.environ.get("N2M_TV_FWD", "1") != "0" and world_size == 1 and not opt.sdf and opt.lambda_tv > 0
                       and not self.tv_split and not self.tv_corners)
        self.adam_tail = os.environ.get("N2M_ADAM_TAIL", "0") == "1" and world_size == 1
        self._tail_ticket = torch.zeros(64 * 32, dtype=torch.int32, device=dev)
        self._mid_events = None
        self.live_first = os.environ.get("N2M_LIVE_FIRST", "0") not in ("0", "")
        self._identity_order = os.environ.get("N2M_LIVE_FIRST", "0") == "2"
        self.lookup_overlap = os.environ.get("N2M_LOOKUP_OVERLAP", "0") == "1" and world_size == 1 and not opt.sdf
        self._fine_ready = None
        if self.lookup_overlap:
            self.s_lookup = L.side_stream(dev, slot=4)
        if os.environ.get("N2M_FILL_DBG"):
            L.call("n2m_debug_fill_times", int(os.environ["N2M_FILL_DBG"]), None)

        e1, e2 = model.encoder, model.encoder_color
        self.rows = e1.embeddings.shape[0]
        self.Lv = e1.num_levels
        self.S = float(np.log2(e1.per_level_scale))
        self.H0 = int(e1.base_resolution)
        self.ho = _host_offsets(e1)
        self.aff = _affine(float(model.bound))
        self.mlp_params = [p for m in (model.sigma_net, model.color_net, model.specular_net) for p in m.parameters()]
        assert len(self.mlp_params) == 7
        self.g1 = torch.empty(self.rows, 1, dtype=torch.float32, device=dev)
        self.g2 = torch.empty(self.rows, 2, dtype=torch.float16, device=dev)
        self.dw = torch.zeros(sum(p.numel() for p in self.mlp_params), dtype=torch.float32, device=dev)
        self.dw_views, o = [], 0
        for p in self.mlp_params:
            self.dw_views.append(self.dw[o:o + p.numel()])
            o += p.numel()
        self._desc = {}
        self._bufs = [None, None, None]
        self._marker = None
        self._last = None
        self._queue = []
        self._prepared = 0
        self.depth = 2
        self._cur = 0

        self._work_cap = (0, 0)
        self._n_spec = int(L.lib().n2m_field_spec_partials())
        self._ticket = torch.zeros(1, dtype=torch.int32, device=dev)
        self._seed = None
        self._aabb = None
        self.shard = False
        if world_size > 1:
            import torch.distributed as dist
            W, split = world_size, int(self.ho[8]) if self.Lv == 16 else 0
            fine = self.rows - split
            peer_mode = os.environ.get("N2M_PEER_STORE", "0") == "1" and not opt.sdf
            cs = split // W
            self._uneven = False
            padded = peer_chunk_rows(split, W, int(os.environ.get("N2M_PEER_PAD_ROWS", "0"))) if peer_mode else None
            if padded is not None:
                cs, even_ok = padded, True
                self._uneven = cs * W != split
            else:
                even_ok = split % W == 0
            ok = self.Lv == 16 and even_ok and fine % W == 0 and os.environ.get("N2M_SHARD_ADAM", "1") != "0"
            if ok:
                self.shard = True
                self._split, self._Cs, self._Fs = split, cs, fine // W
                f32 = lambda *sh: torch.empty(*sh, dtype=torch.float32, device=dev)
                f16 = lambda *sh: torch.empty(*sh, dtype=torch.float16, device=dev)
                self.g1s = {"c": f32(self._Cs, 1), "f": f32(self._Fs, 1)}
                self.g2s = {"c": f16(self._Cs, 2), "f": f16(self._Fs, 2)}
                self._inplace_gather = dist.get_backend() == "nccl"
                self.chunked_gather = os.environ.get("N2M_CHUNKED_GATHER", "1") != "0"
        self._bwd_cfg = (2 if self.shard else 1, float(world_size))
        self.peer = None
        if self.shard and os.environ.get("N2M_PEER_STORE", "0") == "1":
            if opt.sdf:
                raise ValueError("N2M_PEER_STORE covers the NeRF recipes (the SDF head's folded backward is not routed)")
            from .parallel import PeerExchange
            self.peer = PeerExchange(rank, world_size, self.rows, self._split, self._Cs, self._Fs, dev, small_n=self.dw.numel() + 1)
            self._peer_small = torch.empty(self.dw.numel() + 1, dtype=torch.float32, device=dev)
            pk = model.packed_tables()
            self.peer.packed.copy_(pk)
            model._packed = self.peer.packed
            model._packed_buffer = self.peer.packed
            self._peer_route = self.peer.route()
            self._peer_fused = (os.environ.get("N2M_PEER_FUSED", "1") != "0" and self._Cs % 4 == 0 and self._Fs % 4 == 0 and self._split % 2 == 0)
            self._adam_peer = None
        if self.shard:
            self.optimizer.shard_sync = lambda: self.sync_parameters(moments=True)
        self.sdf_fold = os.environ.get("N2M_SDF_FOLD", "1") != "0"
        self.sdf_tv_all = os.environ.get("N2M_SDF_TV_ALL", "1") != "0"
        self.fuse_adam = None
        if world_size == 1 and not opt.sdf and self.Lv == 16 and os.environ.get("N2M_FUSE_ADAM", "0") == "1":
            fl, fr = ctypes.c_uint32(0), ctypes.c_uint32(0)
            self._fuse_cap = 1 << 19
            L.call("n2m_grid_pair_fuse_plan", self._fuse_cap, self.Lv, self.ho.ctypes.data, ctypes.byref(fl), ctypes.byref(fr))
            if fl.value < self.Lv:
                self.fuse_adam = {"first_level": int(fl.value), "first_row": int(fr.value), "alt": None, "desc": {}}
                self._bwd_cfg = (2, 1.0)

    @staticmethod
    def supported(model, opt):
        e1, e2 = model.encoder, model.encoder_color
        sdf = bool(opt.sdf)
        return (bool(getattr(opt, "fused_mlp", False)) and bool(opt.fp16) and getattr(opt, "ind_dim", 0) == 0
                and _affine(float(model.bound)) is not None and same_geometry(e1, e2) and e1.embeddings.shape[1] == 1
                and e2.embeddings.shape[1] == 2 and (sdf or not getattr(opt, "progressive_level", False))
                and opt.patch_size == 1 and (sdf or model.max_level >= e1.num_levels) and not (sdf and opt.lambda_entropy > 0))

    @property
# ... 301 lines not shown
                desc.param[k], desc.grad[k] = p.data_ptr() + off, g.data_ptr()
                desc.exp_avg[k], desc.exp_avg_sq[k] = st["exp_avg"].data_ptr() + off, st["exp_avg_sq"].data_ptr() + off
                desc.half_shadow[k], desc.shadow_mode[k] = pk.data_ptr() + row0 * 8, mode
                desc.numel[k], desc.grad_is_half[k], desc.clear_grad[k] = n * C, is_half, 0
                desc.slot[k] = o._slot[p]
                participants |= 1 << (o._slot[p] - 1)
                groups.append(group_of[p])
                k += 1
        live = set(self.mlp_params[:5]) | (set(self.mlp_params[5:]) if full else set())
        views = dict(zip(self.mlp_params, self.dw_views))
        for p in params:
            if p not in live:
                continue
            st = o.state[p]
            desc.param[k], desc.grad[k] = p.data_ptr(), views[p].data_ptr()
            desc.exp_avg[k], desc.exp_avg_sq[k] = st["exp_avg"].data_ptr(), st["exp_avg_sq"].data_ptr()
            desc.half_shadow[k], desc.shadow_mode[k] = None, 0
            desc.numel[k], desc.grad_is_half[k], desc.clear_grad[k] = p.numel(), 0, 1
            desc.slot[k] = o._slot[p]
            participants |= 1 << (o._slot[p] - 1)
            groups.append(group_of[p])
            k += 1
        desc.count = k
        d = self._desc[key] = (desc, participants, groups)
        return d

    def _gather_packed(self):
        import torch.distributed as dist
        flat = self._packed.view(-1)
        self._gathers = {}
        for h in ("c", "f"):
            row0, n = self._shard_ranges()[h]
            lo = 0 if h == "c" else self._split
            out = flat[lo * 2:(lo + self.world * n) * 2]
            mine = flat[row0 * 2:(row0 + n) * 2]
            self._gathers[h] = dist.all_gather_into_tensor(out, mine if self._inplace_gather else mine.clone(), async_op=True)
        if not self.chunked_gather:
            self._wait_gather()

    def _wait_gather(self, which=("c", "f")):
        g = getattr(self, "_gathers", None)
        if not g:
            return
        for h in which:
            w = g.pop(h, None)
            if w is not None:
                w.wait()

    @torch.no_grad()
    def sync_parameters(self, density_only=False, moments=False):
        if not self.shard:
            return
        self._wait_gather()
        if self.peer is not None:
            self.peer.check()
        done = getattr(self, "_synced", (-1, False, False))
        level = (not density_only, moments)
        if done[0] == self.global_step and (done[1] or density_only) and (done[2] or not moments):
            return
        self._synced = (self.global_step, level[0] or (done[0] == self.global_step and done[1]), level[1] or (done[0] == self.global_step and done[2]))
        import torch.distributed as dist
        e1p, e2p = self.model.encoder.embeddings, self.model.encoder_color.embeddings
        tables = [(e1p.data, 1)] if density_only else [(e1p.data, 1), (e2p.data, 2)]
        if moments:
            for p, C in ((e1p, 1), (e2p, 2)):
                st = self.optimizer.state[p]
                tables += [(st["exp_avg"], C), (st["exp_avg_sq"], C)]
        for t, C in tables:
            flat = t.view(-1)
            for h, (row0, n) in self._shard_ranges().items():
                lo = 0 if h == "c" else self._split
                if h == "c" and getattr(self, "_uneven", False):
                    for r in range(self.world):
                        r0, rn = self._shard_ranges_of(r)["c"]
                        if rn > 0:
                            dist.broadcast(flat[r0 * C:(r0 + rn) * C], src=r)
                    continue
                dist.all_gather_into_tensor(flat[lo * C:(lo + self.world * n) * C], flat[row0 * C:(row0 + n) * C].clone())

    def _optimizer_step(self, full, lr_factor, loss_out=None, fused=None):
        o = self.optimizer
        self._wait_gather()
        desc, participants, groups = self._adam_desc(full, dense_only=fused is not None)
        for k, gi in enumerate(groups):
            desc.lr[k] = float(o.param_groups[gi]["initial_lr"]) * lr_factor
        b1, b2 = o.param_groups[0]["betas"]
        s = L.stream()
        peer_fused = self.peer is not None and self._peer_fused
        scaler_done = False
        if self.lookup_overlap and fused is None and not self.shard and self.Lv == 16:
            d_f, d_c = self._adam_desc_halves(full, lr_factor)
            for d in (d_f, d_c):
                L.call("n2m_adam_step", ctypes.addressof(d), float(b1), float(b2), float(o.param_groups[0]["eps"]), _p(o.scale), _p(o.found_inf),
                       _p(o.bias), s)
                if d is d_f:
                    self._fine_ready = torch.cuda.Event()
                    self._fine_ready.record()
        elif peer_fused:
            if self._adam_peer is None:
                self._adam_peer = self.peer.adam_peer([("s1", "c"), ("s2", "c"), ("s1", "f"), ("s2", "f")] + [None] * (desc.count - 4))
            L.call("n2m_adam_step_peer", ctypes.addressof(desc), float(b1), float(b2), float(o.param_groups[0]["eps"]), _p(o.scale), _p(o.found_inf),
                   _p(o.bias), ctypes.addressof(self._adam_peer), s)
        elif (self.adam_tail and loss_out is not None and fused is None and self.peer is None and not self.shard):
            gf, bf, gi = o.growth
            n_rays, buf, extra = loss_out[:3]
            extra2 = loss_out[3] if len(loss_out) > 3 else None
            ex_buf, ex_scale = extra if extra is not None else (None, 0.0)
            e2_buf, e2_n, e2_scale = extra2 if extra2 is not None else (None, 0, 0.0)
            tail = L.ScalerTail(_p(o.growth_tracker), _p(o.steps), participants, gf, bf, gi, _p(self._w["partial"]), (n_rays + 15) // 16, n_rays,
                                _p(buf), _p(self._loss_sum), _p(ex_buf), self._n_spec, float(ex_scale), _p(e2_buf), int(e2_n), float(e2_scale),
                                _p(self._tail_ticket))
            L.call("n2m_adam_step_scaler", ctypes.addressof(desc), float(b1), float(b2), float(o.param_groups[0]["eps"]), _p(o.scale), _p(o.found_inf),
                   _p(o.bias), ctypes.addressof(tail), s)
            scaler_done = True
        else:
            L.call("n2m_adam_step", ctypes.addressof(desc), float(b1), float(b2), float(o.param_groups[0]["eps"]), _p(o.scale), _p(o.found_inf),
                   _p(o.bias), s)
        self.model.encoder_color._half_version = -1
        if fused is not None:
            L.call("n2m_adam_fuse_restore", ctypes.addressof(fused), self.ho.ctypes.data, self.Lv, _p(o.found_inf), s)
            self._fuse_swap()
        if self.peer is not None:
            for h, (row0, n) in self._shard_ranges().items():
                if peer_fused:
                    self.peer.signal_rows(h)
                else:
                    self.peer.push_rows(h, row0, n)
            self._gathers = self.peer.rows_tokens()
            if not self.chunked_gather:
                self._wait_gather()
        elif self.shard:
            self._gather_packed()
        gf, bf, gi = o.growth
        if scaler_done:
            pass
        elif loss_out is None:
            L.call("n2m_scaler_update_slots", _p(o.scale), _p(o.growth_tracker), _p(o.found_inf), _p(o.steps), _p(o.bias), participants,
                   float(b1), float(b2), gf, bf, gi, s)
        else:
            n_rays, buf, extra = loss_out[:3]
            extra2 = loss_out[3] if len(loss_out) > 3 else None
            ex_buf, ex_scale = extra if extra is not None else (None, 0.0)
            e2_buf, e2_n, e2_scale = extra2 if extra2 is not None else (None, 0, 0.0)
            L.call("n2m_scaler_update_slots_loss3", _p(o.scale), _p(o.growth_tracker), _p(o.found_inf), _p(o.steps), _p(o.bias), participants,
                   float(b1), float(b2), gf, bf, gi, _p(self._w["partial"]), (n_rays + 15) // 16, n_rays, _p(buf), _p(self._loss_sum),
                   _p(ex_buf), self._n_spec, float(ex_scale), _p(e2_buf), int(e2_n), float(e2_scale), s)
        nxt = lr_lambda(self.global_step, self.opt.iters)
        for group in o.param_groups:
            group["lr"] = float(group["initial_lr"]) * nxt

    @torch.no_grad()
    def train_step(self):
        opt, model, dev = self.opt, self.model, self.device
        if not model.training:
            model.train()
        for g in self.optimizer.param_groups:
            g.setdefault("initial_lr", g["lr"])
        if not self._queue:
            self._fill_pipeline()
        b = self._queue.pop(0)
        self.global_step += 1
        assert b.index == self.global_step
        N = b.N
        random_bg = b.bg is not None
        bg = b.bg
        shading = SHADING["diffuse" if (self.global_step < opt.diffuse_step or opt.diffuse_only) else "full"]
        M = self._finish(b)
        self.last_num_points = M
        self.samples_seen += M
        self.rays_seen += N

        if opt.sdf:
            opt.cos_anneal_ratio = min(1, self.global_step / (0.5 * opt.iters))
            opt.normal_anneal_epsilon = 1e-1 * (1 - min(0.999, self.global_step / (0.5 * opt.iters)))
            if opt.progressive_level:
                model.max_level = 4 + int(12 * min(1, self.global_step / (0.5 * opt.iters)))
        w = self._work(max(M, 1), N)
        s = L.stream()
        c = b.cap_m
        xyzs = dirs = ts = None
        if M > 0:
            xyzs, dirs, ts = b.samples[:3 * c], b.samples[3 * c:6 * c], b.samples[6 * c:]
        o = self.optimizer
        pk = model.packed_tables()
        if self.lookup_overlap and getattr(self, "_packed", None) is not None and pk.data_ptr() != self._packed.data_ptr():
            self._fine_ready = None
        sw = self.mlp_params
        e1 = model.encoder
        seed = o.scale if self.world == 1 else o.scale / self.world
        if opt.sdf:
            return self._step_sdf(b, M, N, w, xyzs, dirs, ts, shading, seed, pk)
        fwd_terms = False
        if M > 0:
            fwd = (_p(xyzs), _p(pk), _p(e1.offsets), _p(w["h1"]), _p(w["h2"]), M, self.Lv, self.Lv, self.S, self.H0, e1.gridtype_id,
                   int(bool(e1.align_corners)), e1.interp_id, float(self.aff[0]), float(self.aff[1]))
            if self.shard and getattr(self, "_gathers", None) and self.Lv == 16:
                self._wait_gather(("c",))
                L.call("n2m_grid_encode_forward_packed_levels", *fwd, 0, 8, s)
                self._wait_gather(("f",))
                L.call("n2m_grid_encode_forward_packed_levels", *fwd, 8, 8, s)
            elif self.lookup_overlap and self._fine_ready is not None and self.Lv == 16:
                self.s_lookup.wait_event(self._fine_ready)
                with torch.cuda.stream(self.s_lookup):
                    L.call("n2m_grid_encode_forward_packed_levels", *fwd, 8, 8, L.stream())
                    done = torch.cuda.Event()
                    done.record()
                L.call("n2m_grid_encode_forward_packed_levels", *fwd, 0, 8, s)
                torch.cuda.current_stream(dev).wait_event(done)
            elif self.tv_corners and self.Lv == 16 and self.fuse_adam is None:
                L.call("n2m_grid_encode_forward_packed_tv", *fwd, _p(w["tv4"]), s)
                self._corners_of = (self.global_step, M)
            elif self.tv_fwd and self.Lv == 16 and self.fuse_adam is None:
                L.call("n2m_grid_encode_forward_packed_tvterms", *fwd, float(opt.lambda_tv), float(opt.lambda_tv * (10 if opt.bound > 1 else 1)),
                       float(0.5 / model.bound), _p(seed), _p(w["tv"]), s)
                fwd_terms = True
            else:
                self._wait_gather()
                L.call("n2m_grid_encode_forward_packed", *fwd, s)
            self._mid_step_fill()
            tv_terms = None

            def start_tv():
                go = torch.cuda.Event()
                go.record()
                self.tv_stream.wait_event(go)
                L.grid_backward_config(*self._bwd_cfg)
                with torch.cuda.stream(self.tv_stream):
                    L.call("n2m_grid_tv_terms", _p(xyzs), _p(pk) if self._bwd_cfg[0] == 2 else _p(e1.embeddings), self.ho.ctypes.data, M, self.Lv, self.S, self.H0,
                           e1.gridtype_id, int(bool(e1.align_corners)), e1.interp_id, float(opt.lambda_tv),
                           float(opt.lambda_tv * (10 if opt.bound > 1 else 1)), float(0.5 / model.bound),
                           _p(seed), float(self.aff[0]), float(self.aff[1]), _p(w["tv"]), L.stream())
                    self._tv_done = torch.cuda.Event()
                    self._tv_done.record()
            want_tv = opt.lambda_tv > 0 and self.tv_split and self.Lv == 16
            if want_tv:
                tv_terms = w["tv"]
                if self.tv_at == 0:
                    start_tv()
            elif fwd_terms:
                tv_terms = w["tv"]
                self._tv_done = None
            spec_reg = shading != 0 and opt.lambda_specular > 0
            L.call("n2m_field_forward_train", _p(xyzs), _p(dirs) if shading != 0 else None, _p(w["h1"]), _p(w["h2"]), *[_p(p) for p in sw], M, shading, 1,
                   _p(w["sigma"]), _p(w["rgb"]), None, _p(w["spec_partial"]) if spec_reg else None, s)
            if want_tv and self.tv_at == 1:
                start_tv()
        bg_t, bg_s = (bg, 0.0) if random_bg else (None, 1.0)
        lam_rgb, lam_mask = float(opt.lambda_rgb), float(max(opt.lambda_mask, 0.0))
        early = None
        d_sigma, d_rgb = w["d_sr"][:max(M, 1)], w["d_sr"][max(M, 1):4 * max(M, 1)]
        order = self.live_first and M > 0 and M <= (1 << 20) and self.peer is None
        if order:
            L.call("n2m_composite_live_counts", _p(w["live"]), _p(w["block_live"]))
        try:
            L.call("n2m_composite_loss_train_ent", _p(w["sigma"]), _p(w["rgb"]), _p(ts), _p(b.rays), M, N, 1e-4, _p(b.rgba), _p(bg_t), bg_s, lam_rgb, lam_mask,
                   _p(seed), None, None, _p(d_sigma), _p(d_rgb), _p(w["partial"]), None, None, None, float(max(opt.lambda_entropy, 0.0)), s)
        finally:
            if order:
                L.call("n2m_composite_live_counts", None, None)
        if order:
            L.call("n2m_sample_order_live_first", _p(b.rays), _p(w["live"]), _p(w["block_live"]), N, M, _p(w["perm"]), s)
            if self._identity_order:
                torch.arange(M, dtype=torch.int32, device=dev, out=w["perm"][:M])
        if M > 0:
            if want_tv and self.tv_at == 2:
                start_tv()
            if self.marker_at == 2:
                self._marker = torch.cuda.Event(); self._marker.record()
            L.call("n2m_field_backward_train", _p(xyzs), _p(dirs) if shading != 0 else None, _p(w["h1"]), _p(w["h2"]), *[_p(p) for p in sw], M, shading, 1,
                   _p(d_sigma), _p(d_rgb), None, _p(w["d_h1"]), _p(w["d_h2"]), *[_p(g) for g in self.dw_views], _p(o.found_inf),
                   float(2.0 * opt.lambda_specular / M) if spec_reg else 0.0, _p(seed) if spec_reg else None, s)
            L.grid_backward_config(*self._bwd_cfg)
            need = L.lib().n2m_grid_binned_pair_workspace_bytes(M, self.Lv, self.ho.ctypes.data)
            ws = L.workspace(dev, need)
            tv = opt.lambda_tv > 0
            common = (_p(w["d_h1"]), _p(w["d_h2"]), _p(xyzs), self.ho.ctypes.data, _p(self.g1), _p(self.g2), M,
                      self.Lv, self.Lv, self.S, self.H0, e1.gridtype_id, int(bool(e1.align_corners)), e1.interp_id)
            tail = (_p(o.found_inf), float(self.aff[0]), float(self.aff[1]), 1, _p(ws), ws.numel(), s)
            fused = None
            if self.fuse_adam is not None and M <= self._fuse_cap and tv_terms is None:
                self._adam_desc(shading != 0, dense_only=True)
                fused = self._fuse_desc(lr_lambda(self.global_step - 1, opt.iters))
            if fused is not None:
                tv_args = (_p(pk) if tv else None, float(opt.lambda_tv), float(opt.lambda_tv * (10 if opt.bound > 1 else 1)),
                           float(0.5 / model.bound), _p(seed) if tv else None)
                backward = lambda half: L.call("n2m_grid_encode_backward_binned_pair_adam", *common, *tv_args, *tail[:3], _p(ws), ws.numel(),
                                               ctypes.addressof(fused), s)
            elif tv_terms is not None:
                if self._tv_done is not None:
                    torch.cuda.current_stream(dev).wait_event(self._tv_done)
                backward = lambda half: L.call("n2m_grid_encode_backward_binned_pair_tvt", *common, _p(tv_terms), *tail, half)
            else:
                tv_args = ((_p(pk) if self._bwd_cfg[0] == 2 else _p(e1.embeddings)) if tv else None, float(opt.lambda_tv),
                           float(opt.lambda_tv * (10 if opt.bound > 1 else 1)), float(0.5 / model.bound), _p(seed) if tv else None)
                backward = lambda half: (L.call("n2m_grid_encode_backward_binned_pair", *common, *tv_args, *tail) if half == 0 else
                                         L.call("n2m_grid_encode_backward_binned_pair_half", *common, *tv_args, *tail, half))
            if self.marker_at == 1:
                self._marker = torch.cuda.Event(); self._marker.record()
            if order and fused is None:
                plain_backward = backward

                def backward(half, _b=plain_backward, _perm=w["perm"]):
                    L.call("n2m_grid_backward_sample_order", _p(_perm))
                    try:
                        return _b(half)
                    finally:
                        L.call("n2m_grid_backward_sample_order", None)
            if self.peer is not None:
                self.peer.begin_step()
                L.call("n2m_grid_backward_peer_route", ctypes.byref(self._peer_route))
                try:
                    backward(1)
                    self.peer.signal_grad("f")
                    backward(2)
                    self.peer.signal_grad("c")
                finally:
                    L.call("n2m_grid_backward_peer_route", None)
                early = []
            elif self.shard:
                import torch.distributed as dist
                sp = self._split
                rs = lambda out, src: dist.reduce_scatter_tensor(out.view(-1), src.view(-1), op=dist.ReduceOp.SUM, async_op=True)
                backward(1)
                early = [rs(self.g1s["f"], self.g1[sp:]), rs(self.g2s["f"], self.g2[sp:])]
                backward(2)
                early += [rs(self.g1s["c"], self.g1[:sp]), rs(self.g2s["c"], self.g2[:sp])]
            elif self.sync is not None and self.split_backward and self.Lv == 16:
                split = int(self.ho[8])
                backward(1)
                early = self.sync.all_reduce_sum_begin([self.g1[split:], self.g2[split:]], [])
                backward(2)
            else:
                mid = self.marker_at == 3 and fused is None and tv_terms is None
                if mid:
                    if self._mid_events is None:
                        self._mid_events = [torch.cuda.Event() for _ in range(4)]
                        for e in self._mid_events:
                            e.record()
                    ev = self._mid_events[self.global_step % len(self._mid_events)]
                    L.call("n2m_grid_backward_mid_event", ctypes.c_void_p(ev.cuda_event))
                use_corners = (self.tv_corners and fused is None and tv_terms is None and tv
                               and getattr(self, "_corners_of", None) == (self.global_step, M))
                if use_corners:
                    L.call("n2m_grid_backward_tv_corners", _p(w["tv4"]))
                try:
                    backward(0)
                finally:
                    if use_corners:
                        L.call("n2m_grid_backward_tv_corners", None)
                if mid:
                    self._marker = ev
        else:
            self.g1.zero_()
            self.g2.zero_()
# ... 212 lines not shown
```

### nerf2mesh_amd/network.py

```python
import math
import weakref

import torch
import torch.nn as nn
import torch.nn.functional as F

from .activation import trunc_exp
from .encoding import get_encoder
from .renderer import NeRFRenderer


derived_copy_holders = weakref.WeakSet()


def x_is_cuda(net):
    return net.encoder.embeddings.is_cuda


class MLP(nn.Module):

    def __init__(self, dim_in, dim_out, dim_hidden, num_layers, bias=True):
        super().__init__()
        self.dim_in, self.dim_out, self.dim_hidden, self.num_layers = dim_in, dim_out, dim_hidden, num_layers
        self.net = nn.ModuleList([
            nn.Linear(dim_in if l == 0 else dim_hidden, dim_out if l == num_layers - 1 else dim_hidden, bias=bias)
            for l in range(num_layers)])

    def forward(self, x):
        for l, layer in enumerate(self.net):
            x = layer(x)
            if l != self.num_layers - 1:
                x = F.relu(x, inplace=True)
        return x


class NeRFNetwork(NeRFRenderer):
    def __init__(self, opt, specular_dim=3):
        super().__init__(opt)
        if getattr(opt, "tcnn", False):
            raise NotImplementedError("--tcnn is out of scope (north_star: no tiny-cuda-nn)")
        self.encoder, self.in_dim_density = get_encoder("hashgrid", level_dim=1, desired_resolution=2048 * self.bound, interpolation="linear")
        self.sigma_net = MLP(3 + self.in_dim_density, 1, 32, 2, bias=False)
        self.encoder_color, self.in_dim_color = get_encoder("hashgrid", level_dim=2, desired_resolution=2048 * self.bound, interpolation="linear")
        self.color_net = MLP(3 + self.in_dim_color + self.individual_dim, 3 + specular_dim, 64, 3, bias=False)
        self.encoder_dir, self.in_dim_dir = get_encoder("None")
        self.specular_net = MLP(specular_dim + self.in_dim_dir, 3, 32, 2, bias=False)
        if self.opt.sdf:
            self.register_parameter("variance", nn.Parameter(torch.tensor(0.3, dtype=torch.float32)))
        derived_copy_holders.add(self)

    def packed_tables(self):
        e1, e2 = self.encoder, self.encoder_color
        a, b = e1.embeddings, e2.embeddings
        if a.shape[1] != 1 or b.shape[1] != 2 or a.shape[0] != b.shape[0] or not a.is_cuda:
            return None
        key = (a._version, b._version, a.data_ptr(), b.data_ptr())
        if getattr(self, "_packed_key", None) != key or getattr(self, "_packed", None) is None:
            from .gridencoder import same_geometry
            if not same_geometry(e1, e2):
                return None
            with torch.no_grad():
                pk = getattr(self, "_packed_buffer", None)
                if pk is None or pk.shape != (a.shape[0], 2) or pk.device != a.device:
                    pk = torch.empty(a.shape[0], 2, dtype=torch.float32, device=a.device)
                pk[:, 0] = a.detach()[:, 0]
                pk.view(torch.float16)[:, 2:] = b.detach().half()
            self._packed, self._packed_key = pk, key
        return self._packed

    def invalidate_derived_copies(self):
        self._packed_key = None
        if hasattr(self.encoder_color, "_half_version"):
            self.encoder_color._half_version = -1

    def _can_fuse(self, c=None):
        return bool(getattr(self.opt, "fused_mlp", False)) and c is None and x_is_cuda(self)

    def forward(self, x, d, c=None, shading="full", raw_dirs=False):
        if self._can_fuse(c):
            from .fused import fused_field
            return fused_field(self, x.view(-1, 3), d.view(-1, 3), shading, normalize_dirs=raw_dirs)
        assert not raw_dirs
        sigma = self.density(x)["sigma"]
        color, specular = self.rgb(x, d, c, shading)
        return sigma, color, specular

    def density(self, x):
        if self._can_fuse() and not x.requires_grad:
            from .fused import fused_density
            return {"sigma": fused_density(self, x.reshape(-1, 3)).view(x.shape[:-1])}
        h = self.encoder(x, bound=self.bound, max_level=self.max_level)
        h = self.sigma_net(torch.cat([x, h], dim=-1))
        sigma = h[..., 0].float() if self.opt.sdf else trunc_exp(h[..., 0])
        return {"sigma": sigma}

    def init_double_sphere(self, r1=0.5, r2=1.5, iters=8192, batch_size=8192):
        if not self.opt.sdf:
            return
        opt = torch.optim.Adam(list(self.parameters()), lr=1e-3)
        dev = self.embeddings_device()
        for _ in range(iters):
            xyzs = torch.rand(batch_size, 3, device=dev) * 2 * self.bound - self.bound
            d = torch.norm(xyzs, p=2, dim=-1)
            gt = torch.where(d < (r1 + r2) / 2, d - r1, r2 - d)
            loss = F.mse_loss(self.density(xyzs)["sigma"], gt)
            opt.zero_grad()
            loss.backward()
            opt.step()

    def embeddings_device(self):
        return self.encoder.embeddings.device

    def normal(self, x, epsilon=1e-4):
        M = x.shape[0]
        off = torch.zeros(6, 1, 3, device=x.device, dtype=x.dtype)
        for axis in range(3):
            off[2 * axis, 0, axis] = epsilon
            off[2 * axis + 1, 0, axis] = -epsilon
        pts = (x.unsqueeze(0) + off).clamp(-self.bound, self.bound).reshape(6 * M, 3)
        s = self.density(pts)["sigma"].view(6, M)
        return torch.stack([0.5 * (s[0] - s[1]) / epsilon, 0.5 * (s[2] - s[3]) / epsilon, 0.5 * (s[4] - s[5]) / epsilon], dim=-1)

    def geo_feat(self, x, c=None):
        h = self.encoder_color(x, bound=self.bound, max_level=self.max_level)
        h = torch.cat([x, h], dim=-1)
        if c is not None:
            h = torch.cat([h, c.repeat(x.shape[0], 1) if c.shape[0] == 1 else c], dim=-1)
        return torch.sigmoid(self.color_net(h))

    def rgb(self, x, d, c=None, shading="full"):
        if self._can_fuse(c) and not x.requires_grad:
            from .fused import fused_color
            return fused_color(self, x.reshape(-1, 3), d.reshape(-1, 3), shading)
        geo_feat = self.geo_feat(x, c)
        diffuse = geo_feat[..., :3]
        if shading == "diffuse":
            return diffuse, None
        d = self.encoder_dir(d)
        specular = torch.sigmoid(self.specular_net(torch.cat([d, geo_feat[..., 3:]], dim=-1)))
        color = specular if shading == "specular" else (specular + diffuse).clamp(0, 1)
        return color, specular

    def get_params(self, lr):
        params = super().get_params(lr)
        params.extend([{"params": m.parameters(), "lr": lr}
                       for m in (self.encoder, self.encoder_color, self.sigma_net, self.color_net, self.specular_net)])
        if self.opt.sdf:
            params.append({"params": self.variance, "lr": lr * 0.1})
        return params
```

Measured before the change: 470.9 million samples/s.

## Prebuild fp16 weight LDS image once per step and copy it in field kernels

Adds a persistent fp16 weight image, padded and transposed to the LDS layout, built once per step. It is produced either by a standalone staging kernel or fused into the scaler/loss bookkeeping kernel after the Adam update. The forward and backward field kernels then do a plain uint4 copy of this image into LDS instead of having every block convert and permute the fp32 weights itself. This removes repeated per-block conversion work, at the cost of extra version-key bookkeeping and a risk of using stale weights if invalidation misses a write.

```diff
diff --git a/include/n2m_hip.h b/include/n2m_hip.h
--- a/include/n2m_hip.h
+++ b/include/n2m_hip.h
@@ -474,6 +474,12 @@
                                   float growth_interval, const float* loss_partial, uint32_t n_partial, uint32_t n_rays, float* loss,
                                   float* loss_sum, const float* extra_partial, uint32_t n_extra, float extra_scale,
                                   const float* extra2_partial, uint32_t n_extra2, float extra2_scale, void* stream);
+int n2m_scaler_update_slots_loss3_image(float* scale, float* growth_tracker, float* found_inf, float* steps, float* bias,
+                                        uint32_t participants, double beta1, double beta2, float growth_factor, float backoff_factor,
+                                        float growth_interval, const float* loss_partial, uint32_t n_partial, uint32_t n_rays, float* loss,
+                                        float* loss_sum, const float* extra_partial, uint32_t n_extra, float extra_scale,
+                                        const float* extra2_partial, uint32_t n_extra2, float extra2_scale, const float* const* weights,
+                                        void* image, void* stream);
 
 #define N2M_TAIL_TICKET_WORDS (64 * 32)
 typedef struct {
diff --git a/include/n2m_mlp.h b/include/n2m_mlp.h
--- a/include/n2m_mlp.h
+++ b/include/n2m_mlp.h
@@ -31,6 +31,22 @@
                              float* d_w_spec1, float* found_inf, float spec_reg, const float* seed, void* stream);
 uint32_t n2m_field_spec_partials(void);
 
+uint32_t n2m_field_forward_grid(uint32_t M);
+uint32_t n2m_field_image_halves(void);
+uint32_t n2m_field_image_forward_halves(void);
+int n2m_field_stage_weights(const float* w_sigma0, const float* w_sigma1, const float* w_color0, const float* w_color1,
+                            const float* w_color2, const float* w_spec0, const float* w_spec1, void* image, void* stream);
+int n2m_field_forward_train_img(const float* xyz, const float* dirs, const float* h1, const void* h2, const float* w_sigma0,
+                                const float* w_sigma1, const float* w_color0, const float* w_color1, const float* w_color2,
+                                const float* w_spec0, const float* w_spec1, uint32_t M, int shading, int normalize_dirs, float* sigma, float* rgb,
+                                float* specular, float* spec_sq_partial, const void* image, void* stream);
+int n2m_field_backward_train_img(const float* xyz, const float* dirs, const float* h1, const void* h2, const float* w_sigma0,
+                                 const float* w_sigma1, const float* w_color0, const float* w_color1, const float* w_color2,
+                                 const float* w_spec0, const float* w_spec1, uint32_t M, int shading, int normalize_dirs, const float* d_sigma,
+                                 const float* d_rgb, const float* d_specular, float* d_h1, void* d_h2, float* d_w_sigma0,
+                                 float* d_w_sigma1, float* d_w_color0, float* d_w_color1, float* d_w_color2, float* d_w_spec0,
+                                 float* d_w_spec1, float* found_inf, float spec_reg, const float* seed, const void* image, void* stream);
+
 #ifdef __cplusplus
 }
 #endif
diff --git a/nerf2mesh_amd/_lib.py b/nerf2mesh_amd/_lib.py
--- a/nerf2mesh_amd/_lib.py
+++ b/nerf2mesh_amd/_lib.py
@@ -139,6 +139,8 @@
                                       _vp, _u32, _f32, _vp],
     "n2m_scaler_update_slots_loss3": [_vp, _vp, _vp, _vp, _vp, _u32, ctypes.c_double, ctypes.c_double, _f32, _f32, _f32, _vp, _u32, _u32, _vp, _vp,
                                       _vp, _u32, _f32, _vp, _u32, _f32, _vp],
+    "n2m_scaler_update_slots_loss3_image": [_vp, _vp, _vp, _vp, _vp, _u32, ctypes.c_double, ctypes.c_double, _f32, _f32, _f32, _vp, _u32, _u32, _vp, _vp,
+                                            _vp, _u32, _f32, _vp, _u32, _f32, _vp, _vp, _vp],
     "n2m_sdf_offsets": [_vp, _u32, _f32, _f32, _vp, _vp, _vp],
     "n2m_sdf_alpha_forward": [_vp, _vp, _vp, _vp, _u32, _vp, _f32, _f32, _vp, _vp, _vp, _vp],
     "n2m_sdf_alpha_backward": [_vp, _vp, _vp, _vp, _vp, _u32, _vp, _f32, _f32, _vp, _f32, _vp, _vp, _vp, _vp, _vp, _vp],
@@ -151,6 +153,12 @@
     "n2m_field_forward_train": [_vp] * 11 + [_u32, _int, _int] + [_vp] * 5,
     "n2m_field_backward_train": [_vp] * 11 + [_u32, _int, _int] + [_vp] * 13 + [_f32, _vp, _vp],
     "n2m_field_spec_partials": [],
+    "n2m_field_forward_grid": [_u32],
+    "n2m_field_image_halves": [],
+    "n2m_field_image_forward_halves": [],
+    "n2m_field_stage_weights": [_vp] * 9,
+    "n2m_field_forward_train_img": [_vp] * 11 + [_u32, _int, _int] + [_vp] * 6,
+    "n2m_field_backward_train_img": [_vp] * 11 + [_u32, _int, _int] + [_vp] * 13 + [_f32, _vp, _vp, _vp],
     "n2m_rasterize_forward": [_vp, _vp, _u32, _u32, _u32, _u32, _vp, _vp, _vp],
     "n2m_rasterize_backward": [_vp, _vp, _vp, _vp, _u32, _u32, _u32, _u32, _vp, _vp],
     "n2m_interpolate_forward": [_vp, _vp, _vp, _u32, _u32, _u32, _u32, _u32, _vp, _vp],
@@ -188,7 +196,8 @@
 }
 
 RESTYPES = {"n2m_occupancy_update_partials": _u32, "n2m_grid_binned_workspace_bytes": _u64, "n2m_grid_binned_pair_workspace_bytes": _u64, "n2m_march_fused_workspace_bytes": _u64,
-            "n2m_marching_cubes_workspace_bytes": _u64, "n2m_field_spec_partials": _u32}
+            "n2m_marching_cubes_workspace_bytes": _u64, "n2m_field_spec_partials": _u32,
+            "n2m_field_image_halves": _u32, "n2m_field_forward_grid": _u32, "n2m_field_image_forward_halves": _u32}
 
 F32, F16 = 0, 1
 ADAM_MAX = 16
diff --git a/nerf2mesh_amd/backends/__init__.py b/nerf2mesh_amd/backends/__init__.py
--- a/nerf2mesh_amd/backends/__init__.py
+++ b/nerf2mesh_amd/backends/__init__.py
@@ -100,6 +100,8 @@
             ps = written(self, parameters)
             ids = None if ps is None else {id(p) for p in ps}
             for model in list(derived_copy_holders):
+                if hasattr(model, "field_weights") and (ids is None or any(id(p) in ids for p in model.field_weights())):
+                    model._field_image_key = None
                 if ids is None or id(model.encoder.embeddings) in ids or id(model.encoder_color.embeddings) in ids:
                     model.invalidate_derived_copies()
             return out
diff --git a/nerf2mesh_amd/csrc/mlp.hip b/nerf2mesh_amd/csrc/mlp.hip
--- a/nerf2mesh_amd/csrc/mlp.hip
+++ b/nerf2mesh_amd/csrc/mlp.hip
@@ -2,9 +2,11 @@
 #include <mutex>
 
 #include "n2m_common.hpp"
+#include "n2m_field_image.hpp"
 #include "../../include/n2m_mlp.h"
 
 namespace {
+using namespace n2m_field;
 
 typedef _Float16 h4 __attribute__((ext_vector_type(4)));
 typedef float f16x __attribute__((ext_vector_type(16)));
@@ -13,38 +15,11 @@
 typedef _Float16 h8 __attribute__((ext_vector_type(8)));
 #define MFMA16(a, b, c) __builtin_amdgcn_mfma_f32_32x32x16_f16((a), (b), (c), 0, 0, 0)
 
-constexpr int P_S0 = 28, P_S1 = 36, P_C0 = 44, P_C1 = 68, P_C2 = 68, P_P0 = 12, P_P1 = 36;
-constexpr int P_S1T = 12, P_S0T = 36, P_C2T = 12, P_C1T = 68, P_C0T = 68, P_P1T = 12, P_P0T = 36;
-constexpr int O_S0 = 0;
-constexpr int O_S1 = O_S0 + 32 * P_S0;
-constexpr int O_C0 = O_S1 + 32 * P_S1;
-constexpr int O_C1 = O_C0 + 64 * P_C0;
-constexpr int O_C2 = O_C1 + 64 * P_C1;
-constexpr int O_P0 = O_C2 + 32 * P_C2;
-constexpr int O_P1 = O_P0 + 32 * P_P0;
-constexpr int FWD_HALVES = O_P1 + 32 * P_P1;
-constexpr int O_S1T = FWD_HALVES;
-constexpr int O_S0T = O_S1T + 32 * P_S1T;
-constexpr int O_C2T = O_S0T + 32 * P_S0T;
-constexpr int O_C1T = O_C2T + 64 * P_C2T;
-constexpr int O_C0T = O_C1T + 64 * P_C1T;
-constexpr int O_P1T = O_C0T + 64 * P_C0T;
-constexpr int O_P0T = O_P1T + 32 * P_P1T;
-constexpr int ALL_W_HALVES = O_P0T + 32 * P_P0T;
 constexpr int TILE_PITCH = 68;
 constexpr int TILE_HALVES = 32 * TILE_PITCH;
 constexpr int BWD_HALVES = ALL_W_HALVES + 4 * 2 * TILE_HALVES;
 constexpr int BWD_PC_TILES_HALVES = ALL_W_HALVES + 4 * 4 * TILE_HALVES;
 constexpr int BWD_PC_HALVES = BWD_PC_TILES_HALVES > 65536 ? BWD_PC_TILES_HALVES : 65536;
-
-__device__ __forceinline__ int col_color0(int k) { return k < 32 ? 3 + k : (k < 35 ? k - 32 : -1); }
-__device__ __forceinline__ int col_sigma0(int k) { return k < 16 ? 3 + k : (k < 19 ? k - 16 : -1); }
-__device__ __forceinline__ int col_plain(int k, int in) { return k < in ? k : -1; }
-
-enum Perm { PERM_PLAIN = 0, PERM_COLOR0 = 1, PERM_SIGMA0 = 2 };
-__device__ __forceinline__ int col_of(int perm, int k, int in) {
-    return perm == PERM_COLOR0 ? col_color0(k) : perm == PERM_SIGMA0 ? col_sigma0(k) : col_plain(k, in);
-}
 
 __device__ void stage_w(_Float16* dst, int pitch, const float* __restrict__ W, int out, int in, int m_pad, int k_pad, int perm) {
     for (int idx = threadIdx.x; idx < m_pad * k_pad; idx += blockDim.x) {
@@ -75,6 +50,7 @@
     float* spec_sq_partial;
     float spec_reg;
     const float* seed;
+    const uint4* img;
 };
 constexpr int kSpecPartials = 512;
 
@@ -131,6 +107,23 @@
     __syncthreads();
 }
 
+template <int NT, bool TR>
+__device__ __forceinline__ void copy_images(_Float16* lds, const uint4* __restrict__ img) {
+    constexpr int N = (TR ? ALL_W_HALVES : FWD_HALVES) / 8, PER = (N + NT - 1) / NT;
+    uint4 v[PER];
+#pragma unroll
+    for (int i = 0; i < PER; ++i) {
+        const int e = (int)threadIdx.x + i * NT;
+        v[i] = e < N ? img[e] : make_uint4(0u, 0u, 0u, 0u);
+    }
+#pragma unroll
+    for (int i = 0; i < PER; ++i) {
+        const int e = (int)threadIdx.x + i * NT;
+        if (e < N) reinterpret_cast<uint4*>(lds)[e] = v[i];
+    }
+    __syncthreads();
+}
+
 __device__ __forceinline__ h4 ld_a(const _Float16* W, int pitch, int mb, int kb, int lane) {
     return *reinterpret_cast<const h4*>(W + (32 * mb + (lane & 31)) * pitch + 8 * kb + 4 * (lane >> 5));
 }
@@ -339,7 +332,8 @@
 __global__ void __launch_bounds__(256) field_forward_kernel(FieldArgs a) {
     __builtin_amdgcn_s_setprio(3);
     extern __shared__ __attribute__((aligned(16))) _Float16 lds[];
-    stage_images<256, false, DO_DENSITY, DO_COLOR>(lds, a);
+    if (a.img) copy_images<256, false>(lds, a.img);
+    else stage_images<256, false, DO_DENSITY, DO_COLOR>(lds, a);
 
     const int lane = threadIdx.x & 63, n = lane & 31, g = lane >> 5;
     const uint32_t wave = blockIdx.x * 4 + (threadIdx.x >> 6), n_waves = gridDim.x * 4;
@@ -785,7 +779,8 @@
 __global__ void __launch_bounds__(512) __attribute__((amdgpu_waves_per_eu(2, 2))) field_backward_pc_kernel(FieldArgs a) {
     __builtin_amdgcn_s_setprio(3);
     extern __shared__ __attribute__((aligned(16))) _Float16 lds[];
-    stage_images<512, true, DO_DENSITY, DO_COLOR>(lds, a);
+    if (a.img) copy_images<512, true>(lds, a.img);
+    else stage_images<512, true, DO_DENSITY, DO_COLOR>(lds, a);
 
     const int lane = threadIdx.x & 63, n = lane & 31, g = lane >> 5, wid = threadIdx.x >> 6;
     const int pair = wid & 3;
@@ -1041,7 +1036,7 @@
 static int field_forward_impl(const float* xyz, const float* dirs, const float* h1, const void* h2, const float* w_sigma0,
                                  const float* w_sigma1, const float* w_color0, const float* w_color1, const float* w_color2,
                                  const float* w_spec0, const float* w_spec1, uint32_t M, int shading, int normalize_dirs, float* sigma, float* rgb,
-                                 float* specular, float* spec_sq_partial, void* stream) {
+                                 float* specular, float* spec_sq_partial, const void* image, void* stream) {
     const float* w[7] = {w_sigma0, w_sigma1, w_color0, w_color1, w_color2, w_spec0, w_spec1};
     const bool density = sigma != nullptr;
     if (int rc = check_field("field_forward", xyz, h1, w, density, shading)) return rc;
@@ -1057,6 +1052,7 @@
     for (int i = 0; i < 7; ++i) a.w[i] = w[i];
     a.M = M; a.shading = shading; a.sigma = sigma; a.rgb = rgb; a.specular = specular;
     a.spec_sq_partial = (color && shading != 0) ? spec_sq_partial : nullptr;
+    a.img = (const uint4*)image;
     hipStream_t s = (hipStream_t)stream;
     N2M_PROF_K(N2M_K_MLP_FWD, s, (double)M * (12 + 64 + 4 + (color ? 64 + 12 + 12 + 12 : 0)));
     const size_t smem = (size_t)FWD_HALVES * 2;
@@ -1072,14 +1068,41 @@
                                  const float* w_spec0, const float* w_spec1, uint32_t M, int shading, int normalize_dirs, float* sigma, float* rgb,
                                  float* specular, void* stream) {
     return field_forward_impl(xyz, dirs, h1, h2, w_sigma0, w_sigma1, w_color0, w_color1, w_color2, w_spec0, w_spec1, M, shading, normalize_dirs,
-                              sigma, rgb, specular, nullptr, stream);
+                              sigma, rgb, specular, nullptr, nullptr, stream);
 }
 extern "C" int n2m_field_forward_train(const float* xyz, const float* dirs, const float* h1, const void* h2, const float* w_sigma0,
                                        const float* w_sigma1, const float* w_color0, const float* w_color1, const float* w_color2,
                                        const float* w_spec0, const float* w_spec1, uint32_t M, int shading, int normalize_dirs, float* sigma,
                                        float* rgb, float* specular, float* spec_sq_partial, void* stream) {
     return field_forward_impl(xyz, dirs, h1, h2, w_sigma0, w_sigma1, w_color0, w_color1, w_color2, w_spec0, w_spec1, M, shading, normalize_dirs,
-                              sigma, rgb, specular, spec_sq_partial, stream);
+                              sigma, rgb, specular, spec_sq_partial, nullptr, stream);
+}
+extern "C" int n2m_field_forward_train_img(const float* xyz, const float* dirs, const float* h1, const void* h2, const float* w_sigma0,
+                                           const float* w_sigma1, const float* w_color0, const float* w_color1, const float* w_color2,
+                                           const float* w_spec0, const float* w_spec1, uint32_t M, int shading, int normalize_dirs, float* sigma,
+                                           float* rgb, float* specular, float* spec_sq_partial, const void* image, void* stream) {
+    N2M_REQUIRE(image == nullptr || ((uintptr_t)image & 15u) == 0, N2M_EINVAL, "field_forward_train_img: the image is not 16-byte aligned");
+    return field_forward_impl(xyz, dirs, h1, h2, w_sigma0, w_sigma1, w_color0, w_color1, w_color2, w_spec0, w_spec1, M, shading, normalize_dirs,
+                              sigma, rgb, specular, spec_sq_partial, image, stream);
+}
+
+namespace {
+__global__ void __launch_bounds__(256) field_image_kernel(ImageWeights iw, uint4* __restrict__ image) {
+    const int chunk = blockIdx.x * 256 + threadIdx.x;
+    if (chunk < kImageChunks) image_chunk(iw, image, chunk);
+}
+}
+extern "C" uint32_t n2m_field_forward_grid(uint32_t M) { return persistent_grid(M) * 2; }
+extern "C" uint32_t n2m_field_image_halves(void) { return (uint32_t)ALL_W_HALVES; }
+extern "C" uint32_t n2m_field_image_forward_halves(void) { return (uint32_t)FWD_HALVES; }
+extern "C" int n2m_field_stage_weights(const float* w_sigma0, const float* w_sigma1, const float* w_color0, const float* w_color1,
+                                       const float* w_color2, const float* w_spec0, const float* w_spec1, void* image, void* stream) {
+    ImageWeights iw{{w_sigma0, w_sigma1, w_color0, w_color1, w_color2, w_spec0, w_spec1}};
+    for (int i = 0; i < 7; ++i) N2M_REQUIRE(iw.w[i] != nullptr, N2M_ENULL, "field_stage_weights: weight matrix %d is NULL", i);
+    N2M_REQUIRE(image != nullptr && ((uintptr_t)image & 15u) == 0, N2M_EINVAL, "field_stage_weights: the image is NULL or not 16-byte aligned");
+    N2M_LAUNCH(field_image_kernel, (kImageChunks + 255) / 256, 256, 0, (hipStream_t)stream, iw, (uint4*)image);
+    N2M_CHECK_LAUNCH();
+    return 0;
 }
 extern "C" uint32_t n2m_field_spec_partials(void) { return (uint32_t)kSpecPartials; }
 
@@ -1088,7 +1111,7 @@
                                   const float* w_spec0, const float* w_spec1, uint32_t M, int shading, int normalize_dirs, const float* d_sigma,
                                   const float* d_rgb, const float* d_specular, float* d_h1, void* d_h2, float* d_w_sigma0,
                                   float* d_w_sigma1, float* d_w_color0, float* d_w_color1, float* d_w_color2, float* d_w_spec0,
-                                  float* d_w_spec1, float* found_inf, float spec_reg, const float* seed, void* stream) {
+                                  float* d_w_spec1, float* found_inf, float spec_reg, const float* seed, const void* image, void* stream) {
     const float* w[7] = {w_sigma0, w_sigma1, w_color0, w_color1, w_color2, w_spec0, w_spec1};
     float* dw[7] = {d_w_sigma0, d_w_sigma1, d_w_color0, d_w_color1, d_w_color2, d_w_spec0, d_w_spec1};
     const bool density = d_sigma != nullptr;
@@ -1128,6 +1151,7 @@
         float* part = dw_scratch(s);
         N2M_REQUIRE(part != nullptr, (int)hipErrorOutOfMemory, "field_backward: no memory for the weight-gradient scratch");
         a.dw_partial = part;
+        a.img = (const uint4*)image;
         if (color && density) N2M_LAUNCH((field_backward_pc_kernel<true, true>), grid, 512, smem, s, a);
         else if (color) N2M_LAUNCH((field_backward_pc_kernel<false, true>), grid, 512, smem, s, a);
         else N2M_LAUNCH((field_backward_pc_kernel<true, false>), grid, 512, smem, s, a);
@@ -1155,7 +1179,7 @@
                                   float* d_w_spec1, float* found_inf, void* stream) {
     return field_backward_impl(xyz, dirs, h1, h2, w_sigma0, w_sigma1, w_color0, w_color1, w_color2, w_spec0, w_spec1, M, shading, normalize_dirs,
                                d_sigma, d_rgb, d_specular, d_h1, d_h2, d_w_sigma0, d_w_sigma1, d_w_color0, d_w_color1, d_w_color2, d_w_spec0,
-                               d_w_spec1, found_inf, 0.f, nullptr, stream);
+                               d_w_spec1, found_inf, 0.f, nullptr, nullptr, stream);
 }
 extern "C" int n2m_field_backward_train(const float* xyz, const float* dirs, const float* h1, const void* h2, const float* w_sigma0,
                                         const float* w_sigma1, const float* w_color0, const float* w_color1, const float* w_color2,
@@ -1165,5 +1189,17 @@
                                         float* d_w_spec0, float* d_w_spec1, float* found_inf, float spec_reg, const float* seed, void* stream) {
     return field_backward_impl(xyz, dirs, h1, h2, w_sigma0, w_sigma1, w_color0, w_color1, w_color2, w_spec0, w_spec1, M, shading, normalize_dirs,
                                d_sigma, d_rgb, d_specular, d_h1, d_h2, d_w_sigma0, d_w_sigma1, d_w_color0, d_w_color1, d_w_color2, d_w_spec0,
-                               d_w_spec1, found_inf, spec_reg, seed, stream);
-}
+                               d_w_spec1, found_inf, spec_reg, seed, nullptr, stream);
+}
+extern "C" int n2m_field_backward_train_img(const float* xyz, const float* dirs, const float* h1, const void* h2, const float* w_sigma0,
+                                            const float* w_sigma1, const float* w_color0, const float* w_color1, const float* w_color2,
+                                            const float* w_spec0, const float* w_spec1, uint32_t M, int shading, int normalize_dirs,
+                                            const float* d_sigma, const float* d_rgb, const float* d_specular, float* d_h1, void* d_h2,
+                                            float* d_w_sigma0, float* d_w_sigma1, float* d_w_color0, float* d_w_color1, float* d_w_color2,
+                                            float* d_w_spec0, float* d_w_spec1, float* found_inf, float spec_reg, const float* seed,
+                                            const void* image, void* stream) {
+    N2M_REQUIRE(image == nullptr || ((uintptr_t)image & 15u) == 0, N2M_EINVAL, "field_backward_train_img: the image is not 16-byte aligned");
+    return field_backward_impl(xyz, dirs, h1, h2, w_sigma0, w_sigma1, w_color0, w_color1, w_color2, w_spec0, w_spec1, M, shading, normalize_dirs,
+                               d_sigma, d_rgb, d_specular, d_h1, d_h2, d_w_sigma0, d_w_sigma1, d_w_color0, d_w_color1, d_w_color2, d_w_spec0,
+                               d_w_spec1, found_inf, spec_reg, seed, image, stream);
+}
diff --git a/nerf2mesh_amd/csrc/n2m_field_image.hpp b/nerf2mesh_amd/csrc/n2m_field_image.hpp
--- /dev/null
+++ b/nerf2mesh_amd/csrc/n2m_field_image.hpp
@@ -0,0 +1,68 @@
+#pragma once
+#include <stdint.h>
+
+namespace n2m_field {
+
+constexpr int P_S0 = 28, P_S1 = 36, P_C0 = 44, P_C1 = 68, P_C2 = 68, P_P0 = 12, P_P1 = 36;
+constexpr int P_S1T = 12, P_S0T = 36, P_C2T = 12, P_C1T = 68, P_C0T = 68, P_P1T = 12, P_P0T = 36;
+constexpr int O_S0 = 0;
+constexpr int O_S1 = O_S0 + 32 * P_S0;
+constexpr int O_C0 = O_S1 + 32 * P_S1;
+constexpr int O_C1 = O_C0 + 64 * P_C0;
+constexpr int O_C2 = O_C1 + 64 * P_C1;
+constexpr int O_P0 = O_C2 + 32 * P_C2;
+constexpr int O_P1 = O_P0 + 32 * P_P0;
+constexpr int FWD_HALVES = O_P1 + 32 * P_P1;
+constexpr int O_S1T = FWD_HALVES;
+constexpr int O_S0T = O_S1T + 32 * P_S1T;
+constexpr int O_C2T = O_S0T + 32 * P_S0T;
+constexpr int O_C1T = O_C2T + 64 * P_C2T;
+constexpr int O_C0T = O_C1T + 64 * P_C1T;
+constexpr int O_P1T = O_C0T + 64 * P_C0T;
+constexpr int O_P0T = O_P1T + 32 * P_P1T;
+constexpr int ALL_W_HALVES = O_P0T + 32 * P_P0T;
+static_assert(FWD_HALVES % 8 == 0 && ALL_W_HALVES % 8 == 0, "the images are copied in 16-byte pieces");
+
+__device__ __forceinline__ int col_color0(int k) { return k < 32 ? 3 + k : (k < 35 ? k - 32 : -1); }
+__device__ __forceinline__ int col_sigma0(int k) { return k < 16 ? 3 + k : (k < 19 ? k - 16 : -1); }
+__device__ __forceinline__ int col_plain(int k, int in) { return k < in ? k : -1; }
+
+enum Perm { PERM_PLAIN = 0, PERM_COLOR0 = 1, PERM_SIGMA0 = 2 };
+__device__ __forceinline__ int col_of(int perm, int k, int in) {
+    return perm == PERM_COLOR0 ? col_color0(k) : perm == PERM_SIGMA0 ? col_sigma0(k) : col_plain(k, in);
+}
+
+struct ImageRegion { int off, rows, pitch, mat, out, in, perm, tr; };
+constexpr int kImageRegions = 14;
+__device__ constexpr ImageRegion kRegions[kImageRegions] = {
+    {O_S0, 32, P_S0, 0, 32, 19, PERM_SIGMA0, 0}, {O_S1, 32, P_S1, 1, 1, 32, PERM_PLAIN, 0},   {O_C0, 64, P_C0, 2, 64, 35, PERM_COLOR0, 0},
+    {O_C1, 64, P_C1, 3, 64, 64, PERM_PLAIN, 0},  {O_C2, 32, P_C2, 4, 6, 64, PERM_PLAIN, 0},   {O_P0, 32, P_P0, 5, 32, 6, PERM_PLAIN, 0},
+    {O_P1, 32, P_P1, 6, 3, 32, PERM_PLAIN, 0},
+    {O_S1T, 32, P_S1T, 1, 1, 32, PERM_PLAIN, 1}, {O_S0T, 32, P_S0T, 0, 32, 19, PERM_SIGMA0, 1}, {O_C2T, 64, P_C2T, 4, 6, 64, PERM_PLAIN, 1},
+    {O_C1T, 64, P_C1T, 3, 64, 64, PERM_PLAIN, 1}, {O_C0T, 64, P_C0T, 2, 64, 35, PERM_COLOR0, 1}, {O_P1T, 32, P_P1T, 6, 3, 32, PERM_PLAIN, 1},
+    {O_P0T, 32, P_P0T, 5, 32, 6, PERM_PLAIN, 1},
+};
+
+struct ImageWeights { const float* w[7]; };
+
+__device__ __forceinline__ _Float16 image_half(const ImageWeights& iw, int i) {
+    int r = 0;
+#pragma unroll
+    for (int j = 1; j < kImageRegions; ++j) r += i >= kRegions[j].off ? 1 : 0;
+    const ImageRegion g = kRegions[r];
+    const int e = i - g.off, row = e / g.pitch, c = e - row * g.pitch;
+    const int m = g.tr ? c : row, k = g.tr ? row : c;
+    const int col = col_of(g.perm, k, g.in);
+    return (m < g.out && col >= 0) ? (_Float16)iw.w[g.mat][m * g.in + col] : (_Float16)0.0f;
+}
+
+__device__ __forceinline__ void image_chunk(const ImageWeights& iw, uint4* __restrict__ image, int chunk) {
+    typedef _Float16 h8_t __attribute__((ext_vector_type(8)));
+    h8_t v;
+#pragma unroll
+    for (int j = 0; j < 8; ++j) v[j] = image_half(iw, chunk * 8 + j);
+    image[chunk] = __builtin_bit_cast(uint4, v);
+}
+constexpr int kImageChunks = ALL_W_HALVES / 8;
+
+}
diff --git a/nerf2mesh_amd/csrc/step_helpers.hip b/nerf2mesh_amd/csrc/step_helpers.hip
--- a/nerf2mesh_amd/csrc/step_helpers.hip
+++ b/nerf2mesh_amd/csrc/step_helpers.hip
@@ -1,6 +1,7 @@
 #include <string.h>
 
 #include "n2m_common.hpp"
+#include "n2m_field_image.hpp"
 #include "../../include/n2m_peer.h"
 
 namespace {
@@ -1207,6 +1208,44 @@
     return 0;
 }
 
+__global__ void __launch_bounds__(256) scaler_update_slots_image_kernel(float* scale, float* growth_tracker, float* found_inf, float* steps, float* bias,
+                                                 uint32_t participants, double beta1, double beta2, float growth_factor, float backoff_factor,
+                                                 float growth_interval, const float* __restrict__ loss_partial, uint32_t n_partial, float inv_rays,
+                                                 float* __restrict__ loss, float* __restrict__ loss_sum, const float* __restrict__ extra_partial,
+                                                 uint32_t n_extra, float extra_scale, const float* __restrict__ extra2_partial, uint32_t n_extra2,
+                                                 float extra2_scale, n2m_field::ImageWeights iw, uint4* __restrict__ image) {
+    __builtin_amdgcn_s_setprio(3);
+    if (blockIdx.x != 0) {
+        const int chunk = ((int)blockIdx.x - 1) * 256 + (int)threadIdx.x;
+        if (chunk < n2m_field::kImageChunks) n2m_field::image_chunk(iw, image, chunk);
+        return;
+    }
+    scaler_update_slots_body<false>(scale, growth_tracker, found_inf, steps, bias, participants, beta1, beta2, growth_factor, backoff_factor, growth_interval,
+                             loss_partial, n_partial, inv_rays, loss, loss_sum, extra_partial, n_extra, extra_scale, extra2_partial, n_extra2, extra2_scale);
+}
+extern "C" int n2m_scaler_update_slots_loss3_image(float* scale, float* growth_tracker, float* found_inf, float* steps, float* bias,
+                                                   uint32_t participants, double beta1, double beta2, float growth_factor, float backoff_factor,
+                                                   float growth_interval, const float* loss_partial, uint32_t n_partial, uint32_t n_rays, float* loss,
+                                                   float* loss_sum, const float* extra_partial, uint32_t n_extra, float extra_scale,
+                                                   const float* extra2_partial, uint32_t n_extra2, float extra2_scale, const float* const* weights,
+                                                   void* image, void* stream) {
+    N2M_REQUIRE(found_inf != nullptr && steps != nullptr && bias != nullptr, N2M_ENULL, "scaler_update_slots: NULL found_inf / steps / bias");
+    N2M_REQUIRE(loss_partial != nullptr && n_rays > 0, N2M_EINVAL, "scaler_update_slots_loss: needs the loss partials and the ray count");
+    N2M_REQUIRE(weights != nullptr && image != nullptr && ((uintptr_t)image & 15u) == 0, N2M_EINVAL,
+                "scaler_update_slots_loss3_image: needs the seven weight pointers and a 16-byte aligned image");
+    n2m_field::ImageWeights iw;
+    for (int i = 0; i < 7; ++i) {
+        N2M_REQUIRE(weights[i] != nullptr, N2M_ENULL, "scaler_update_slots_loss3_image: weight matrix %d is NULL", i);
+        iw.w[i] = weights[i];
+    }
+    scaler_update_slots_image_kernel<<<1 + (n2m_field::kImageChunks + 255) / 256, 256, 0, (hipStream_t)stream>>>(
+        scale, growth_tracker, found_inf, steps, bias, participants, beta1, beta2, growth_factor, backoff_factor, growth_interval, loss_partial, n_partial,
+        1.0f / (float)n_rays, loss, loss_sum, extra_partial, extra_partial ? n_extra : 0u, extra_scale, extra2_partial, extra2_partial ? n_extra2 : 0u,
+        extra2_scale, iw, (uint4*)image);
+    N2M_CHECK_LAUNCH();
+    return 0;
+}
+
 extern "C" int n2m_scaler_update_slots_loss2(float* scale, float* growth_tracker, float* found_inf, float* steps, float* bias,
                                              uint32_t participants, double beta1, double beta2, float growth_factor, float backoff_factor,
                                              float growth_interval, const float* loss_partial, uint32_t n_partial, uint32_t n_rays, float* loss,
diff --git a/nerf2mesh_amd/engine.py b/nerf2mesh_amd/engine.py
--- a/nerf2mesh_amd/engine.py
+++ b/nerf2mesh_amd/engine.py
@@ -124,6 +124,8 @@
         self.aff = _affine(float(model.bound))
         self.mlp_params = [p for m in (model.sigma_net, model.color_net, model.specular_net) for p in m.parameters()]
         assert len(self.mlp_params) == 7
+        self.use_field_image = os.environ.get("N2M_FIELD_IMAGE", "1") != "0" and hasattr(model, "field_image")
+        self._image_weights = None
         self.g1 = torch.empty(self.rows, 1, dtype=torch.float32, device=dev)
         self.g2 = torch.empty(self.rows, 2, dtype=torch.float16, device=dev)
         self.dw = torch.zeros(sum(p.numel() for p in self.mlp_params), dtype=torch.float32, device=dev)
@@ -591,6 +593,8 @@
         o = self.optimizer
         self._wait_gather()
         desc, participants, groups = self._adam_desc(full, dense_only=fused is not None)
+        img = self.model._field_image if (self.use_field_image and getattr(self.model, "_field_image_key", None) is not None) else None
+        self.model._field_image_key = None
         for k, gi in enumerate(groups):
             desc.lr[k] = float(o.param_groups[gi]["initial_lr"]) * lr_factor
         b1, b2 = o.param_groups[0]["betas"]
@@ -651,9 +655,17 @@
             extra2 = loss_out[3] if len(loss_out) > 3 else None
             ex_buf, ex_scale = extra if extra is not None else (None, 0.0)
             e2_buf, e2_n, e2_scale = extra2 if extra2 is not None else (None, 0, 0.0)
-            L.call("n2m_scaler_update_slots_loss3", _p(o.scale), _p(o.growth_tracker), _p(o.found_inf), _p(o.steps), _p(o.bias), participants,
-                   float(b1), float(b2), gf, bf, gi, _p(self._w["partial"]), (n_rays + 15) // 16, n_rays, _p(buf), _p(self._loss_sum),
-                   _p(ex_buf), self._n_spec, float(ex_scale), _p(e2_buf), int(e2_n), float(e2_scale), s)
+            book = (_p(o.scale), _p(o.growth_tracker), _p(o.found_inf), _p(o.steps), _p(o.bias), participants,
+                    float(b1), float(b2), gf, bf, gi, _p(self._w["partial"]), (n_rays + 15) // 16, n_rays, _p(buf), _p(self._loss_sum),
+                    _p(ex_buf), self._n_spec, float(ex_scale), _p(e2_buf), int(e2_n), float(e2_scale))
+            if img is not None:
+                ptrs = [p.data_ptr() for p in self.mlp_params]
+                if self._image_weights is None or list(self._image_weights) != ptrs:
+                    self._image_weights = (ctypes.c_void_p * 7)(*ptrs)
+                L.call("n2m_scaler_update_slots_loss3_image", *book, ctypes.addressof(self._image_weights), _p(img), s)
+                self.model._field_image_key = tuple(v for p in self.mlp_params for v in (p._version, p.data_ptr()))
+            else:
+                L.call("n2m_scaler_update_slots_loss3", *book, s)
         nxt = lr_lambda(self.global_step, self.opt.iters)
         for group in o.param_groups:
             group["lr"] = float(group["initial_lr"]) * nxt
@@ -695,6 +707,7 @@
         if self.lookup_overlap and getattr(self, "_packed", None) is not None and pk.data_ptr() != self._packed.data_ptr():
             self._fine_ready = None
         sw = self.mlp_params
+        img = model.field_image() if self.use_field_image else None
         e1 = model.encoder
         seed = o.scale if self.world == 1 else o.scale / self.world
         if opt.sdf:
@@ -750,8 +763,8 @@
                 tv_terms = w["tv"]
                 self._tv_done = None
             spec_reg = shading != 0 and opt.lambda_specular > 0
-            L.call("n2m_field_forward_train", _p(xyzs), _p(dirs) if shading != 0 else None, _p(w["h1"]), _p(w["h2"]), *[_p(p) for p in sw], M, shading, 1,
-                   _p(w["sigma"]), _p(w["rgb"]), None, _p(w["spec_partial"]) if spec_reg else None, s)
+            L.call("n2m_field_forward_train_img", _p(xyzs), _p(dirs) if shading != 0 else None, _p(w["h1"]), _p(w["h2"]), *[_p(p) for p in sw], M, shading, 1,
+                   _p(w["sigma"]), _p(w["rgb"]), None, _p(w["spec_partial"]) if spec_reg else None, _p(img), s)
             if want_tv and self.tv_at == 1:
                 start_tv()
         bg_t, bg_s = (bg, 0.0) if random_bg else (None, 1.0)
@@ -776,9 +789,9 @@
                 start_tv()
             if self.marker_at == 2:
                 self._marker = torch.cuda.Event(); self._marker.record()
-            L.call("n2m_field_backward_train", _p(xyzs), _p(dirs) if shading != 0 else None, _p(w["h1"]), _p(w["h2"]), *[_p(p) for p in sw], M, shading, 1,
+            L.call("n2m_field_backward_train_img", _p(xyzs), _p(dirs) if shading != 0 else None, _p(w["h1"]), _p(w["h2"]), *[_p(p) for p in sw], M, shading, 1,
                    _p(d_sigma), _p(d_rgb), None, _p(w["d_h1"]), _p(w["d_h2"]), *[_p(g) for g in self.dw_views], _p(o.found_inf),
-                   float(2.0 * opt.lambda_specular / M) if spec_reg else 0.0, _p(seed) if spec_reg else None, s)
+                   float(2.0 * opt.lambda_specular / M) if spec_reg else 0.0, _p(seed) if spec_reg else None, _p(img), s)
             L.grid_backward_config(*self._bwd_cfg)
             need = L.lib().n2m_grid_binned_pair_workspace_bytes(M, self.Lv, self.ho.ctypes.data)
             ws = L.workspace(dev, need)
diff --git a/nerf2mesh_amd/network.py b/nerf2mesh_amd/network.py
--- a/nerf2mesh_amd/network.py
+++ b/nerf2mesh_amd/network.py
@@ -68,8 +68,28 @@
             self._packed, self._packed_key = pk, key
         return self._packed
 
+    def field_weights(self):
+        return [l.weight for m in (self.sigma_net, self.color_net, self.specular_net) for l in m.net]
+
+    def field_image(self):
+        ws = self.field_weights()
+        key = tuple(v for p in ws for v in (p._version, p.data_ptr()))
+        if getattr(self, "_field_image_key", None) != key or getattr(self, "_field_image", None) is None:
+            from . import _lib as L
+            shapes = [(32, 19), (1, 32), (64, 35), (64, 64), (6, 64), (32, 6), (3, 32)]
+            if not all(p.is_cuda and p.dtype == torch.float32 and p.is_contiguous() and tuple(p.shape) == sh for p, sh in zip(ws, shapes)):
+                return None
+            img = getattr(self, "_field_image", None)
+            if img is None or img.device != ws[0].device:
+                img = torch.empty(int(L.lib().n2m_field_image_halves()), dtype=torch.int16, device=ws[0].device)
+            with torch.cuda.device(ws[0].device):
+                L.call("n2m_field_stage_weights", *[L.ptr(p) for p in ws], L.ptr(img), L.stream())
+            self._field_image, self._field_image_key = img, key
+        return self._field_image
+
     def invalidate_derived_copies(self):
         self._packed_key = None
+        self._field_image_key = None
         if hasattr(self.encoder_color, "_half_version"):
             self.encoder_color._half_version = -1
 
```

New measurement: 475.7 million samples/s (median of 6 runs). 1.01x the previous value.
